# Soltanilara/av-aloha

Measured on AMD Instinct MI355X. Metric: env-steps/sec (whole node) at 4096 parallel envs, SlotInsertion-3Arms, higher is better.
Workload: dtype f32

## Files before the change

av_aloha_amd/build.py:

```python
import os
import subprocess
import sys

HERE = os.path.dirname(os.path.abspath(__file__))
ROOT = os.path.dirname(HERE)
LIB = os.path.join(HERE, "libavsim.so")
SRC = os.path.join(HERE, "csrc")


def _stale(target, sources):
    if not os.path.exists(target):
        return True
    t = os.path.getmtime(target)
    return any(os.path.getmtime(s) > t for s in sources)


def build_hip(force=False, verbose=False):
    srcs = [os.path.join(SRC, f) for f in sorted(os.listdir(SRC)) if not f.endswith(".o") and not f.startswith(".")] + [os.path.join(ROOT, "include", "avsim.h"), os.path.abspath(__file__)]
    if not force and not _stale(LIB, srcs):
        return LIB
    import fcntl
    with open(os.path.join(SRC, ".build.lock"), "w") as lock:
        fcntl.flock(lock, fcntl.LOCK_EX)
        if not force and not _stale(LIB, srcs):
            return LIB
        return _build_hip_locked(verbose)


def _build_hip_locked(verbose):
    hipcc = os.environ.get("HIPCC", "/opt/rocm/bin/hipcc")
    common = [hipcc, "--offload-arch=gfx950", "-std=c++17", "-fPIC", "-fno-gpu-rdc", "-c"]
    units = [
        ("avsim_api", ["-O2", "-fno-hip-fp32-correctly-rounded-divide-sqrt", "-fgpu-flush-denormals-to-zero", "-fno-slp-vectorize", "-fno-vectorize",
                       "-mllvm", "-amdgpu-atomic-optimizer-strategy=None", "-mllvm", "-amdgpu-sched-strategy=max-ilp"] + (["-DAVSIM_RENDER_STATS"] if os.environ.get("AVSIM_RENDER_STATS") else []) + os.environ.get("AVSIM_EXTRA_FLAGS", "").split()),
        ("avsim_phys_f64", ["-O3", "-ffp-contract=off", "-mllvm", "-amdgpu-sched-strategy=max-ilp"] + os.environ.get("AVSIM_EXTRA_FLAGS_F64", "").split()),
    ]
    procs = []
    for name, extra in units:
        cmd = common + extra + ["-o", os.path.join(SRC, name + ".o"), os.path.join(SRC, name + ".hip")]
        if verbose:
            print(" ".join(cmd), file=sys.stderr)
        procs.append((cmd, subprocess.Popen(cmd)))
    for cmd, p in procs:
        if p.wait() != 0:
            raise subprocess.CalledProcessError(p.returncode, cmd)
    tmp = LIB + ".tmp%d" % os.getpid()
    link = [hipcc, "--offload-arch=gfx950", "-shared", "-fPIC", "-fno-gpu-rdc", "-o", tmp] + [os.path.join(SRC, n + ".o") for n, _ in units]
    if verbose:
        print(" ".join(link).replace(tmp, LIB), file=sys.stderr)
    subprocess.check_call(link)
    os.replace(tmp, LIB)
    return LIB


def build_oracle(force=False):
    d = os.path.join(ROOT, "oracle")
    so = os.path.join(d, "liborc.so")
    srcs = [os.path.join(d, f) for f in os.listdir(d) if f.endswith((".c", ".h"))]
    if force or _stale(so, srcs):
        subprocess.check_call(["make", "-C", d, "-B", "liborc.so"], stdout=subprocess.DEVNULL)
    return so


if __name__ == "__main__":
    print(build_hip(force="--force" in sys.argv, verbose=True))
    print(build_oracle(force="--force" in sys.argv))
```

av_aloha_amd/csrc/avsim_api.hip:

```cpp
#include <hip/hip_runtime.h>

#include <cmath>
#include <cstdarg>
#include <cstdio>
#include <cstdlib>
#include <cstring>
#include <memory>
#include <string>
#include <thread>
#include <vector>

#include "../../include/avsim.h"
#include "avsim_compose.hip.h"
#include "avsim_imgprep.hip.h"
#include "avsim_episode.hip.h"
#include "avsim_ik.hip.h"
#include "avsim_jpeg.hip.h"
#include "avsim_model.h"
#include "avsim_phys.hip.h"
#include "avsim_render.hip.h"
#include "avsim_vis.hip.h"

using namespace avs;

// ... 452 lines not shown
    if (!std::strcmp(name, "render_cam_major")) { h->vis.cam_major = value != 0; return AVSIM_OK; }
    if (!std::strcmp(name, "render_chunk")) { if (value < 1) { h->set_error("render_chunk is a number of envs >= 1"); return AVSIM_EINVAL; } h->render.env_chunk = (int)value; return AVSIM_OK; }
    if (!std::strcmp(name, "jpeg_decode_events")) { h->jpegdec_events = value != 0; return AVSIM_OK; }
    if (!std::strcmp(name, "jpeg_decode_budget")) { if (value < 1) { h->set_error("jpeg_decode_budget is a number of bytes >= 1"); return AVSIM_EINVAL; } h->jpegdec.coef_budget = (size_t)value; return AVSIM_OK; }
    if (!std::strcmp(name, "diffik_iters")) { h->ik.diff_iters = (int)value; return AVSIM_OK; }
    if (!std::strcmp(name, "gradik_iters")) { h->ik.grad_iters = (int)value; return AVSIM_OK; }
    try {
        if (h->phys.set_option(name, value)) {
            if (!std::strcmp(name, "num_joints")) h->nj = (int)value;
            return AVSIM_OK;
        }
    } catch (const std::exception& ex) {
        h->set_error("avsim_set_option(%s): %s", name, ex.what());
        return AVSIM_EHIP;
    }
    h->set_error("avsim_set_option: unknown option '%s'", name);
    return AVSIM_EINVAL;
}

int avsim_sync(avsim_t* h) {
    if (!h) return AVSIM_EINVAL;
    AVS_ON_DEVICE(h);
    HIPCHK(h, hipStreamSynchronize(h->stream));
    return AVSIM_OK;
}

int avsim_set_stream(avsim_t* h, void* s) {
    if (!h) return AVSIM_EINVAL;
    AVS_ON_DEVICE(h);
    HIPCHK(h, hipStreamSynchronize(h->stream));
    if (h->own_stream && h->stream) (void)hipStreamDestroy(h->stream);
    h->stream = (hipStream_t)s;
    h->own_stream = false;
    return AVSIM_OK;
}

int avsim_event_record(avsim_t* h, int slot) {
    if (!h || slot < 0 || slot >= 16) return AVSIM_EINVAL;
    AVS_ON_DEVICE(h);
    HIPCHK(h, hipEventRecord(h->ev[slot], h->stream));
    return AVSIM_OK;
}

int avsim_event_elapsed_ms(avsim_t* h, int a, int b, float* ms) {
    if (!h || !ms || a < 0 || a >= 16 || b < 0 || b >= 16) return AVSIM_EINVAL;
    AVS_ON_DEVICE(h);
    HIPCHK(h, hipEventSynchronize(h->ev[b]));
    HIPCHK(h, hipEventElapsedTime(ms, h->ev[a], h->ev[b]));
    return AVSIM_OK;
}

int avsim_kernel_time(avsim_t* h, int reset, double* total_ms, int64_t* launches) {
    if (!h) return AVSIM_EINVAL;
    AVS_ON_DEVICE(h);
    double tot = 0;
    for (size_t i = 0; i + 1 < h->kev_used; i += 2) {
        float ms = 0;
        HIPCHK(h, hipEventSynchronize(h->kev[i + 1]));
        HIPCHK(h, hipEventElapsedTime(&ms, h->kev[i], h->kev[i + 1]));
        tot += ms;
    }
    if (total_ms) *total_ms = tot + h->kev_ms;
    if (launches) *launches = (int64_t)(h->kev_used / 2) + h->kev_n;
    if (reset) { h->kev_used = 0; h->kev_ms = 0; h->kev_n = 0; }
    return AVSIM_OK;
}

int avsim_render_kernel_time(avsim_t* h, int reset, double* total_ms, int64_t* launches) {
    if (!h) return AVSIM_EINVAL;
    AVS_ON_DEVICE(h);
    double tot = 0;
    for (size_t i = 0; i + 1 < h->render.tev_used; i += 2) {
        float ms = 0;
        HIPCHK(h, hipEventSynchronize(h->render.tev[i + 1]));
        HIPCHK(h, hipEventElapsedTime(&ms, h->render.tev[i], h->render.tev[i + 1]));
        tot += ms;
    }
    if (total_ms) *total_ms = tot + h->render.tev_ms;
    if (launches) *launches = (int64_t)(h->render.tev_used / 2) + h->render.tev_n;
    if (reset) { h->render.tev_used = 0; h->render.tev_ms = 0; h->render.tev_n = 0; }
    return AVSIM_OK;
}

int avsim_observe(avsim_t* h, double* agent_pos, int32_t* reward, uint8_t* success) {
    if (!h) return AVSIM_EINVAL;
    AVS_ON_DEVICE(h);
    int rc;
    void *dap = nullptr, *drw = nullptr, *dsu = nullptr;
    size_t N = h->N;
    if (agent_pos && (rc = h->out_begin(4, agent_pos, sizeof(double) * N * h->nj, &dap))) return rc;
    if (reward && (rc = h->out_begin(5, reward, sizeof(int32_t) * N, &drw))) return rc;
    if (success && (rc = h->out_begin(6, success, N, &dsu))) return rc;
    h->phys.force_reward = 1;
    rc = h->phys.launch(h->stream, h->N, 0, nullptr, h->nj, h->d_qpos, h->d_qvel, h->d_ctrl, h->d_warm, h->d_latch, (double*)dap, (int32_t*)drw,
                        (uint8_t*)dsu, h->err);
    h->phys.force_reward = 0;
    if (rc) return rc;
    if ((rc = h->out_end(4, agent_pos, sizeof(double) * N * h->nj))) return rc;
    if ((rc = h->out_end(5, reward, sizeof(int32_t) * N))) return rc;
    if ((rc = h->out_end(6, success, N))) return rc;
    return h->finish();
}

int avsim_fk_jac(avsim_t* h, int arm, int n, const double* q, double* T, double* J) {
    if (!h || arm < 0 || arm > 2 || n <= 0 || !q) { if (h) h->set_error("avsim_fk_jac: bad arguments"); return AVSIM_EINVAL; }
    AVS_ON_DEVICE(h);
    int nj = h->ik.arm[arm].n, rc;
    const void* dq;
    void *dT = nullptr, *dJ = nullptr;
    if ((rc = h->in(0, q, sizeof(double) * n * nj, &dq))) return rc;
    if (T && (rc = h->out_begin(1, T, sizeof(double) * n * 16, &dT))) return rc;
    if (J && (rc = h->out_begin(2, J, sizeof(double) * n * 6 * nj, &dJ))) return rc;
    dim3 grid((n + 63) / 64);
    if (nj == 6) hipLaunchKernelGGL(k_fk_jac<6>, grid, dim3(64), 0, h->stream, h->ik, arm, n, (const double*)dq, (double*)dT, (double*)dJ);
    else hipLaunchKernelGGL(k_fk_jac<7>, grid, dim3(64), 0, h->stream, h->ik, arm, n, (const double*)dq, (double*)dT, (double*)dJ);
    HIPCHK(h, hipGetLastError());
    if ((rc = h->out_end(1, T, sizeof(double) * n * 16))) return rc;
    if ((rc = h->out_end(2, J, sizeof(double) * n * 6 * nj))) return rc;
    return h->finish();
}

int avsim_ik(avsim_t* h, int arm, int controller, int max_iters, int n, const double* q, const double* pos,
             const double* quat, double* qout) {
    if (!h || arm < 0 || arm > 2 || n <= 0 || !q || !pos || !quat || !qout || controller < 0 || controller > 1) {
        if (h) h->set_error("avsim_ik: bad arguments");
        return AVSIM_EINVAL;
    }
    if (controller == 1 && arm == 2) { h->set_error("avsim_ik: GradIK is defined for the 6-DoF manipulators only"); return AVSIM_EINVAL; }
    AVS_ON_DEVICE(h);
    int nj = h->ik.arm[arm].n, rc;
    int iters = max_iters > 0 ? max_iters : (controller == 0 ? h->ik.diff_iters : h->ik.grad_iters);
    const void *dq, *dp, *dqt;
    void* dout;
    if ((rc = h->in(0, q, sizeof(double) * n * nj, &dq))) return rc;
    if ((rc = h->in(1, pos, sizeof(double) * n * 3, &dp))) return rc;
    if ((rc = h->in(2, quat, sizeof(double) * n * 4, &dqt))) return rc;
    if ((rc = h->out_begin(3, qout, sizeof(double) * n * nj, &dout))) return rc;
    dim3 grid(controller == 1 ? (n + 3) / 4 : (n + 63) / 64);
    if (nj == 6)
        hipLaunchKernelGGL(k_ik<6>, grid, dim3(64), 0, h->stream, h->ik, arm, controller, iters, n, (const double*)dq, (const double*)dp,
                           (const double*)dqt, (double*)dout);
    else
        hipLaunchKernelGGL(k_ik<7>, grid, dim3(64), 0, h->stream, h->ik, arm, controller, iters, n, (const double*)dq, (const double*)dp,
                           (const double*)dqt, (double*)dout);
    HIPCHK(h, hipGetLastError());
    if ((rc = h->out_end(3, qout, sizeof(double) * n * nj))) return rc;
    return h->finish();
}

}

template <typename real>
static int reset_impl(avsim_t* h, const uint8_t* mask, const double* obj) {
    int rc;
    const void *dm = nullptr, *dobj;
    if (mask && (rc = h->in(0, mask, h->N, &dm))) return rc;
    if ((rc = h->in(1, obj, sizeof(double) * h->N * h->nobj * 7, &dobj))) return rc;
    hipLaunchKernelGGL(k_reset<real>, dim3((h->N + 63) / 64), dim3(64), 0, h->stream, h->N, h->nq, h->nv, h->nu, h->nobj,
                       (const unsigned char*)dm, (const double*)dobj, h->phys.d_qpos_home, h->phys.d_ctrl_home, h->phys.d_obj_qadr,
                       (real*)h->d_qpos, (real*)h->d_qvel, (real*)h->d_ctrl, (real*)h->d_warm, h->d_latch, h->phys.d_obj_reset);
    HIPCHK(h, hipGetLastError());
    if ((rc = h->phys.launch(h->stream, h->N, 0, nullptr, h->nj, h->d_qpos, h->d_qvel, h->d_ctrl, h->d_warm, h->d_latch, nullptr, nullptr,
                             nullptr, h->err)))
        return rc;
    return h->finish();
}

extern "C" {

int avsim_reset(avsim_t* h, const uint8_t* mask, const double* obj_qpos) {
    if (!h || !obj_qpos) { if (h) h->set_error("avsim_reset: obj_qpos is required"); return AVSIM_EINVAL; }
    AVS_ON_DEVICE(h);
    h->state_ver++;
    return h->f64 ? reset_impl<double>(h, mask, obj_qpos) : reset_impl<float>(h, mask, obj_qpos);
}

static int step_common(avsim_t* h, const float* d_action, int nsub, double* agent_pos, int32_t* reward, uint8_t* success) {
    int rc;
    h->state_ver++;
    void *dap = nullptr, *drw = nullptr, *dsu = nullptr;
    size_t N = h->N;
    if (agent_pos && (rc = h->out_begin(4, agent_pos, sizeof(double) * N * h->nj, &dap))) return rc;
    if (reward && (rc = h->out_begin(5, reward, sizeof(int32_t) * N, &drw))) return rc;
    if (success && (rc = h->out_begin(6, success, N, &dsu))) return rc;
    if (h->ktiming) {
        if (h->kev_used >= 2 * EV_RING) {
            for (size_t i = 0; i + 1 < h->kev_used; i += 2) {
                float ms = 0;
                HIPCHK(h, hipEventSynchronize(h->kev[i + 1]));
                HIPCHK(h, hipEventElapsedTime(&ms, h->kev[i], h->kev[i + 1]));
                h->kev_ms += ms;
            }
            h->kev_n += (int64_t)(h->kev_used / 2);
            h->kev_used = 0;
        }
        while (h->kev.size() < h->kev_used + 2) { hipEvent_t e; HIPCHK(h, hipEventCreate(&e)); h->kev.push_back(e); }
        HIPCHK(h, hipEventRecord(h->kev[h->kev_used], h->stream));
    }
    if ((rc = h->phys.launch(h->stream, h->N, nsub, d_action, h->nj, h->d_qpos, h->d_qvel, h->d_ctrl, h->d_warm, h->d_latch, (double*)dap,
                             (int32_t*)drw, (uint8_t*)dsu, h->err)))
        return rc;
    if (h->ktiming) {
        HIPCHK(h, hipEventRecord(h->kev[h->kev_used + 1], h->stream));
        h->kev_used += 2;
    }
    if ((rc = h->out_end(4, agent_pos, sizeof(double) * N * h->nj))) return rc;
    if ((rc = h->out_end(5, reward, sizeof(int32_t) * N))) return rc;
    if ((rc = h->out_end(6, success, N))) return rc;
    return h->finish();
}

int avsim_step(avsim_t* h, const float* action, int nsub, double* agent_pos, int32_t* reward, uint8_t* success) {
    if (!h || !action || nsub < 0) { if (h) h->set_error("avsim_step: bad arguments"); return AVSIM_EINVAL; }
    AVS_ON_DEVICE(h);
    const void* da;
    int rc;
    if ((rc = h->in(0, action, sizeof(float) * h->N * h->nj, &da))) return rc;
    return step_common(h, (const float*)da, nsub, agent_pos, reward, success);
}

int avsim_step_ctrl(avsim_t* h, int nsub, double* agent_pos, int32_t* reward, uint8_t* success) {
    if (!h || nsub < 0) { if (h) h->set_error("avsim_step_ctrl: bad arguments"); return AVSIM_EINVAL; }
    AVS_ON_DEVICE(h);
    return step_common(h, nullptr, nsub, agent_pos, reward, success);
}

int avsim_step_cartesian(avsim_t* h, const double* action23, int ik_mode, int nsub, double* agent_pos, int32_t* reward,
                         uint8_t* success) {
    if (!h || !action23 || nsub < 0 || (ik_mode != AVSIM_IK_REFERENCE && ik_mode != AVSIM_IK_DLS)) {
        if (h) h->set_error("avsim_step_cartesian: bad arguments");
        return AVSIM_EINVAL;
    }
    if (h->num_arms != 3) { h->set_error("avsim_step_cartesian: the 23-D Cartesian action drives three arms (sim_env.py:277-282)"); return AVSIM_EINVAL; }
    AVS_ON_DEVICE(h);
    const void* da;
    int rc;
    if ((rc = h->in(0, action23, sizeof(double) * h->N * 23, &da))) return rc;
    auto launch = [&](dim3 grid, int arm0) {
        if (h->f64)
            hipLaunchKernelGGL(k_cart_ctrl<double>, grid, dim3(64), 0, h->stream, h->ik, ik_mode, arm0, h->N, h->nq, h->nu, (const double*)da,
                               (const double*)h->d_qpos, (double*)h->d_ctrl);
        else
            hipLaunchKernelGGL(k_cart_ctrl<float>, grid, dim3(64), 0, h->stream, h->ik, ik_mode, arm0, h->N, h->nq, h->nu, (const double*)da,
                               (const float*)h->d_qpos, (float*)h->d_ctrl);
    };
    if (ik_mode == AVSIM_IK_DLS) launch(dim3((h->N + 63) / 64, 3), 0);
    else {
        if (h->f64) hipLaunchKernelGGL(k_gradik_ctrl<double>, dim3((h->N + 3) / 4, 2), dim3(64), 0, h->stream, h->ik, h->N, h->nq, h->nu, (const double*)da, (const double*)h->d_qpos, (double*)h->d_ctrl);
        else hipLaunchKernelGGL(k_gradik_ctrl<float>, dim3((h->N + 3) / 4, 2), dim3(64), 0, h->stream, h->ik, h->N, h->nq, h->nu, (const double*)da, (const float*)h->d_qpos, (float*)h->d_ctrl);
        launch(dim3((h->N + 63) / 64, 1), 2);
    }
    HIPCHK(h, hipGetLastError());
    return step_common(h, nullptr, nsub, agent_pos, reward, success);
}

static int put(avsim_t* h, int slot, const double* src, void* dst, size_t n) {
    if (!src) return 0;
    const void* d;
    int rc;
    if ((rc = h->in(slot, src, sizeof(double) * n, &d))) return rc;
    unsigned g = (unsigned)((n + 255) / 256);
    if (h->f64) hipLaunchKernelGGL((k_convert<double, double>), dim3(g), dim3(256), 0, h->stream, n, (const double*)d, (double*)dst);
    else hipLaunchKernelGGL((k_convert<double, float>), dim3(g), dim3(256), 0, h->stream, n, (const double*)d, (float*)dst);
    return 0;
}
static int get(avsim_t* h, int slot, double* dst, const void* src, size_t n) {
    if (!dst) return 0;
    void* d;
    int rc;
    if ((rc = h->out_begin(slot, dst, sizeof(double) * n, &d))) return rc;
    unsigned g = (unsigned)((n + 255) / 256);
    if (h->f64) hipLaunchKernelGGL((k_convert<double, double>), dim3(g), dim3(256), 0, h->stream, n, (const double*)src, (double*)d);
    else hipLaunchKernelGGL((k_convert<float, double>), dim3(g), dim3(256), 0, h->stream, n, (const float*)src, (double*)d);
    return h->out_end(slot, dst, sizeof(double) * n);
}

int avsim_get_state(avsim_t* h, double* qpos, double* qvel, double* ctrl, double* warm) {
    if (!h) return AVSIM_EINVAL;
    AVS_ON_DEVICE(h);
    size_t N = h->N;
    int rc;
    if ((rc = get(h, 0, qpos, h->d_qpos, N * h->nq))) return rc;
    if ((rc = get(h, 1, qvel, h->d_qvel, N * h->nv))) return rc;
    if ((rc = get(h, 2, ctrl, h->d_ctrl, N * h->nu))) return rc;
    if ((rc = get(h, 3, warm, h->d_warm, N * h->nv))) return rc;
    HIPCHK(h, hipGetLastError());
    return h->finish();
}

int avsim_set_state(avsim_t* h, const double* qpos, const double* qvel, const double* ctrl, const double* warm) {
    if (!h) return AVSIM_EINVAL;
    AVS_ON_DEVICE(h);
    h->state_ver++;
    size_t N = h->N;
    int rc;
    if ((rc = put(h, 0, qpos, h->d_qpos, N * h->nq))) return rc;
    if ((rc = put(h, 1, qvel, h->d_qvel, N * h->nv))) return rc;
    if ((rc = put(h, 2, ctrl, h->d_ctrl, N * h->nu))) return rc;
    if ((rc = put(h, 3, warm, h->d_warm, N * h->nv))) return rc;
    HIPCHK(h, hipGetLastError());
    if ((rc = h->phys.launch(h->stream, h->N, 0, nullptr, h->nj, h->d_qpos, h->d_qvel, h->d_ctrl, h->d_warm, h->d_latch, nullptr, nullptr,
                             nullptr, h->err)))
        return rc;
    return h->finish();
}

int avsim_get_latch(avsim_t* h, int32_t* latch) {
    if (!h || !latch) return AVSIM_EINVAL;
    AVS_ON_DEVICE(h);
    HIPCHK(h, hipMemcpyAsync(latch, h->d_latch, sizeof(int32_t) * (size_t)h->N, h->io_device ? hipMemcpyDeviceToDevice : hipMemcpyDeviceToHost, h->stream));
    return h->finish();
}

int avsim_set_latch(avsim_t* h, const int32_t* latch) {
    if (!h || !latch) return AVSIM_EINVAL;
    AVS_ON_DEVICE(h);
    HIPCHK(h, hipMemcpyAsync(h->d_latch, latch, sizeof(int32_t) * (size_t)h->N, h->io_device ? hipMemcpyDeviceToDevice : hipMemcpyHostToDevice, h->stream));
    return h->finish();
}

int avsim_get_reset_poses(avsim_t* h, double* obj_qpos) {
    if (!h || !obj_qpos) return AVSIM_EINVAL;
    AVS_ON_DEVICE(h);
    HIPCHK(h, hipMemcpyAsync(obj_qpos, h->phys.d_obj_reset, sizeof(double) * (size_t)h->N * h->nobj * 7, h->io_device ? hipMemcpyDeviceToDevice : hipMemcpyDeviceToHost, h->stream));
    return h->finish();
}

int avsim_set_reset_poses(avsim_t* h, const double* obj_qpos) {
    if (!h || !obj_qpos) return AVSIM_EINVAL;
    AVS_ON_DEVICE(h);
    HIPCHK(h, hipMemcpyAsync(h->phys.d_obj_reset, obj_qpos, sizeof(double) * (size_t)h->N * h->nobj * 7, h->io_device ? hipMemcpyDeviceToDevice : hipMemcpyHostToDevice, h->stream));
    return h->finish();
}

int avsim_set_qpos(avsim_t* h, const double* qpos) {
    if (!h || !qpos) return AVSIM_EINVAL;
    return avsim_set_state(h, qpos, nullptr, nullptr, nullptr);
}

int avsim_get_contacts(avsim_t* h, int32_t* ncon, int32_t* pairs, double* dist) {
    if (!h) return AVSIM_EINVAL;
    AVS_ON_DEVICE(h);
    size_t N = h->N, cap = h->phys.maxcon;
    if (h->io_device) {
        if (ncon) HIPCHK(h, hipMemcpyAsync(ncon, h->phys.d_ncon, N * 4, hipMemcpyDeviceToDevice, h->stream));
        if (pairs) HIPCHK(h, hipMemcpyAsync(pairs, h->phys.d_cpairs, N * cap * 8, hipMemcpyDeviceToDevice, h->stream));
        if (dist) HIPCHK(h, hipMemcpyAsync(dist, h->phys.d_cdist, N * cap * 8, hipMemcpyDeviceToDevice, h->stream));
        return AVSIM_OK;
    }
    HIPCHK(h, hipStreamSynchronize(h->stream));
    if (ncon) HIPCHK(h, hipMemcpy(ncon, h->phys.d_ncon, N * 4, hipMemcpyDeviceToHost));
    if (pairs) HIPCHK(h, hipMemcpy(pairs, h->phys.d_cpairs, N * cap * 8, hipMemcpyDeviceToHost));
    if (dist) HIPCHK(h, hipMemcpy(dist, h->phys.d_cdist, N * cap * 8, hipMemcpyDeviceToHost));
    return AVSIM_OK;
}

int avsim_get_phase_cycles(avsim_t* h, int64_t* out) {
    if (!h || !out || !h->phys.d_prof) return AVSIM_EINVAL;
    AVS_ON_DEVICE(h);
    HIPCHK(h, hipStreamSynchronize(h->stream));
    HIPCHK(h, hipMemcpy(out, h->phys.d_prof, (size_t)h->N * avs::PROF_W * 8, h->io_device ? hipMemcpyDeviceToDevice : hipMemcpyDeviceToHost));
    return AVSIM_OK;
}

int avsim_get_diag(avsim_t* h, int32_t* diag) {
    if (!h || !diag) return AVSIM_EINVAL;
    AVS_ON_DEVICE(h);
    size_t N = h->N;
    if (h->io_device) {
        HIPCHK(h, hipMemcpyAsync(diag, h->phys.d_diag, N * 16, hipMemcpyDeviceToDevice, h->stream));
        return AVSIM_OK;
    }
    HIPCHK(h, hipStreamSynchronize(h->stream));
    HIPCHK(h, hipMemcpy(diag, h->phys.d_diag, N * 16, hipMemcpyDeviceToHost));
    return AVSIM_OK;
// ... 497 lines not shown
```

av_aloha_amd/csrc/avsim_newton.hip.h:

```cpp
#pragma once
#include "avsim_math.hip.h"

namespace avs {

typedef float nv4f __attribute__((ext_vector_type(4)));
typedef double nv2d __attribute__((ext_vector_type(2)));
AVS_DEV void load_row16(GLB_PTR(const float) src, float* v) {
    GLB_PTR(const nv4f) p = (GLB_PTR(const nv4f))src;
    nv4f a = p[0], b = p[1], c = p[2], d = p[3];
    asm volatile("" : "+v"(a), "+v"(b), "+v"(c), "+v"(d));
    v[0] = a.x; v[1] = a.y; v[2] = a.z; v[3] = a.w; v[4] = b.x; v[5] = b.y; v[6] = b.z; v[7] = b.w;
    v[8] = c.x; v[9] = c.y; v[10] = c.z; v[11] = c.w; v[12] = d.x; v[13] = d.y; v[14] = d.z; v[15] = d.w;
}
AVS_DEV void load_row16(GLB_PTR(const double) src, double* v) {
    GLB_PTR(const nv2d) p = (GLB_PTR(const nv2d))src;
    nv2d t[8];
#pragma unroll
    for (int q = 0; q < 8; q++) t[q] = p[q];
    asm volatile("" : "+v"(t[0]), "+v"(t[1]), "+v"(t[2]), "+v"(t[3]), "+v"(t[4]), "+v"(t[5]), "+v"(t[6]), "+v"(t[7]));
#pragma unroll
    for (int q = 0; q < 8; q++) { v[2 * q] = t[q].x; v[2 * q + 1] = t[q].y; }
}

template <typename real>
// ... 491 lines not shown
    const int nv = A.nv;
    NComp c;
    c.mydof = lane < nv ? lane : nv; c.nc = nv; c.oa0 = 0; c.on = 0; c.oact = false;
    if (A.ntree > 8 || whole) return c;
    unsigned mine = 0;
    for (int i = lane; i < ne; i += 64) {
        const int ra = A.rowI[i];
        if (((ra >> 19) & 15) != 0) mine |= (1u << ((ra >> 10) & 7)) | (1u << ((ra >> 23) & 7));
    }
    unsigned tmask = 0;
#pragma unroll
    for (int t = 0; t < 8; t++) tmask |= __any((mine >> t) & 1u) ? (1u << t) : 0u;
    const bool isc = lane < nv && ((tmask >> A.dof_tree[lane < nv ? lane : 0]) & 1u);
    const unsigned long long cm = __ballot(isc);
    c.nc = __popcll(cm);
    if (c.nc == nv) return c;
    if (isc) tmp[__popcll(cm & ((1ull << lane) - 1ull))] = lane;
    NSYNC();
    c.mydof = lane < c.nc ? tmp[lane] : nv;
    NSYNC();
    const int t = lane >> 3;
    c.oact = t < A.ntree && !((tmask >> t) & 1u);
    c.oa0 = c.oact ? A.tree_dofadr[t] : 0;
    c.on = c.oact ? A.tree_dofnum[t] : 0;
    return c;
}

template <typename real, bool FWD>
AVS_DEV void ncomp_subst(const NewtonArgs<real>& A, const NComp& c, int lane) {
    const int nv = A.nv, nc = c.nc, i8 = lane & 7;
    const bool omine = c.oact && i8 < c.on;
    const int a0 = c.oa0, obase = (a0 + i8) * (a0 + i8 + 1) / 2 + a0;
    real ocf[TREE_W];
#pragma unroll
    for (int k = 0; k < TREE_W; k++) {
        const bool in = FWD ? (omine && k < i8) : (omine && k < c.on && k > i8);
        const real v = A.H[in ? (FWD ? obase + k : (a0 + k) * (a0 + k + 1) / 2 + a0 + i8) : 0];
        ocf[k] = in ? v : real(0);
    }
    const real odg = A.H[omine ? obase + i8 : 0];
    const real odinv = omine ? real(1) / odg : real(1);
    const real og = A.g[omine ? a0 + i8 : 0];
    real ox = omine ? (FWD ? -og : og) : real(0);
    const int md = c.mydof, rb = md * (md + 1) / 2;
    const bool cm = lane < nc;
    const real cg = A.g[cm ? md : 0];
    real x = cm ? (FWD ? -cg : cg) : real(0);
    const real dinv = cm ? real(1) / A.H[rb + md] : real(0);
    if (nc < nv) {
#pragma unroll
        for (int jj = 0; jj < TREE_W; jj++) {
            const int j = FWD ? jj : TREE_W - 1 - jj;
            const real xj = oct_bcast_n(ox * odinv, j);
            ox = i8 == j ? xj : ox - ocf[j] * xj;
        }
    }
    if (FWD) {
        int cn = __builtin_amdgcn_readlane(md, 0);
        real Lnext = (lane > 0 && cm) ? A.H[rb + cn] : real(0);
        for (int j = 0; j < nc; j++) {
            const real Lc = Lnext;
            if (j + 1 < nc) { cn = __builtin_amdgcn_readlane(md, j + 1); Lnext = (lane > j + 1 && cm) ? A.H[rb + cn] : real(0); }
            const real yj = lane_get(x * dinv, j);
            if (lane == j) x = yj;
            else if (lane > j) x -= Lc * yj;
        }
    } else {
        int cn = __builtin_amdgcn_readlane(md, nc - 1);
        real Lnext = lane < nc - 1 ? A.H[cn * (cn + 1) / 2 + md] : real(0);
        for (int i = nc - 1; i >= 0; i--) {
            const real Lc = Lnext;
            if (i > 0) { cn = __builtin_amdgcn_readlane(md, i - 1); Lnext = lane < i - 1 ? A.H[cn * (cn + 1) / 2 + md] : real(0); }
            const real xi = lane_get(x * dinv, i);
            if (lane == i) x = xi;
            else if (lane < i) x -= Lc * xi;
        }
    }
    NSYNC();
    LDS_PTR(real) out = FWD ? A.g : A.dl;
    if (cm) out[md] = x;
    if (nc < nv && omine) out[a0 + i8] = ox;
}

template <typename real, int NCH, bool COUPLED>
__device__ __attribute__((always_inline)) int newton_solve(KPtr<real> ka, GLB_PTR(const real) rows, LDS_PTR(real) r_, LDS_PTR(int) ii_, LDS_PTR(const int) li_, int nefc, int ncon, int nlead,
                                                      int iters, real tol, real scale, int profiling) {
    const int lane = threadIdx.x & 63;
    NewtonArgs<real> A;
    {
        LDS_PTR(real) r = (LDS_PTR(real))(unsigned long long)(unsigned)__builtin_amdgcn_readfirstlane((int)(unsigned)(unsigned long long)r_);
        LDS_PTR(int) ii = (LDS_PTR(int))(unsigned long long)(unsigned)__builtin_amdgcn_readfirstlane((int)(unsigned)(unsigned long long)ii_);
        LDS_PTR(const int) li = (LDS_PTR(const int))(unsigned long long)(unsigned)__builtin_amdgcn_readfirstlane((int)(unsigned)(unsigned long long)li_);
        tol = lane_get(tol, 0); scale = lane_get(scale, 0);
        const Layout __attribute__((address_space(4)))* L = &ka->lay;
        const MOff __attribute__((address_space(4)))* O = &ka->mo;
        A.rowS = r + L->rowS; A.rowI = ii + L->rowI; A.rmeta = ii + L->rmeta;
        {
            const unsigned long long p_ = (unsigned long long)rows;
            A.rJ = (GLB_PTR(const real))(((unsigned long long)(unsigned)__builtin_amdgcn_readfirstlane((int)(unsigned)(p_ >> 32)) << 32) | (unsigned)__builtin_amdgcn_readfirstlane((int)(unsigned)p_));
        }
        A.M = r + L->M; A.a = r + L->qacc; A.as = r + L->asm_;
        A.H = r + L->nH; A.g = r + L->ng; A.dl = r + L->ndl; A.jv = r + L->njv;
        A.cefc = ii + L->cefc;
        A.prof = profiling ? ii + L->nprof : (LDS_PTR(int))nullptr;
        A.tree_dofadr = li + O->tree_dofadr; A.tree_dofnum = li + O->tree_dofnum; A.tree_madr = li + O->tree_madr; A.dof_tree = li + O->dof_tree;
        A.nv = __builtin_amdgcn_readfirstlane(ka->m.nv); A.ntree = __builtin_amdgcn_readfirstlane(ka->m.ntree);
        A.nefc = __builtin_amdgcn_readfirstlane(nefc); A.ncon = __builtin_amdgcn_readfirstlane(ncon);
        A.nlead = __builtin_amdgcn_readfirstlane(nlead); A.iters = __builtin_amdgcn_readfirstlane(iters);
        A.tol = tol; A.scale = scale; A.ls_tol = ka->m.ls_tolerance; A.ls_iters = __builtin_amdgcn_readfirstlane(ka->m.ls_iterations);
        A.early_exit = __builtin_amdgcn_readfirstlane(ka->m.newton_early_exit);
    }
    const int nv = A.nv, ne = A.nefc;
    {
        const int k = lane < nv ? lane : 0, t = A.dof_tree[k];
        A.k_a0 = A.tree_dofadr[t]; A.k_n = A.tree_dofnum[t]; A.k_mb = A.tree_madr[t] + (k - A.k_a0) * A.k_n;
    }
    int used = 0;
    constexpr bool coupled = COUPLED;
    NComp comp;
    if constexpr (coupled) comp = ncomponent<real>(A, lane, ne, (LDS_PTR(int))A.dl, __builtin_amdgcn_readfirstlane(ka->m.newton_component) == 0);
    long long tp0 = A.prof ? __builtin_readcyclecounter() : 0;
    NCon<real> con[NCH];
#pragma unroll
    for (int ch = 0; ch < NCH; ch++) {
        NCon<real>& c = con[ch];
        const int ci = ch * 64 + lane;
        const int ce = ci < A.ncon ? A.cefc[ci] : -1;
        c.head = ce >= 0 ? (ce & 0xffff) : -1;
        c.dim = ce >= 0 ? (ce >> 16) : 0;
        c.mu = 0; c.Dm = 0;
#pragma unroll
        for (int j = 0; j < 6; j++) { c.S[j] = 0; c.D[j] = 0; }
        if (c.head >= 0) {
#pragma unroll
            for (int j = 0; j < 6; j++)
                if (j < c.dim) { c.D[j] = real(1) / A.rowS[RS_S * (c.head + j) + 1]; if (j > 0) c.S[j] = real(1) / A.rowS[RS_S * (c.head + j) + 7]; }
            if (c.dim > 1) {
                const real R0 = A.rowS[RS_S * c.head + 1], R1 = A.rowS[RS_S * (c.head + 1) + 1];
                c.mu = c.S[1] * sqrt(R1 / R0);
                c.S[0] = c.mu;
                c.Dm = (real(1) / R0) / tmax(real(1e-15), c.mu * c.mu * (1 + c.mu * c.mu));
            }
        }
    }
    const bool jar_ready = true;
    {
        const real c1 = ncost<real, NCH>(A, lane, con, A.as, 8, false);
        const real c0 = ncost<real, NCH>(A, lane, con, (LDS_PTR(const real))A.a, 2);
        if (!(c0 < c1)) {
            for (int k = lane; k < nv; k += 64) A.a[k] = A.as[k];
            for (int i = lane; i < ne; i += 64) A.rowS[RS_S * i + 2] = A.rowS[RS_S * i + 8];
        }
        NSYNC();
    }
    NPROF(0);
    int zone[NCH];
    real cw[NCH][6], cc1[NCH][6], cc2[NCH][6], cs1[NCH], cs2[NCH];
    bool have_L = false;
    unsigned long long sig_lead = 0, sig_z1[NCH];
#pragma unroll
    for (int ch = 0; ch < NCH; ch++) sig_z1[ch] = 0;
    bool forces_current = false, quad_step = false;
    unsigned long long prev_lead = 0, prev_sgn = 0, prev_z1[NCH];
#pragma unroll
    for (int ch = 0; ch < NCH; ch++) prev_z1[ch] = 0;
    real alpha_prev = 0;
    for (int it = 0; it < A.iters; it++) {
        used++;
        if (it > 0) {
            for (int i = lane; i < ne; i += 64) A.rowS[RS_S * i + 2] += alpha_prev * A.jv[i];
            NSYNC();
        } else if (!jar_ready) {
            for (int i = lane; i < ne; i += 64) A.rowS[RS_S * i + 2] = nrow_dot(A, i, (LDS_PTR(const real))A.a) - A.rowS[RS_S * i];
            NSYNC();
        }
        for (int i = lane; i < A.nlead; i += 64) {
            real f, h;
            nrow_scalar<real>(A.rmeta[i] & 3, A.rowS[RS_S * i + 2], A.rowS[RS_S * i + 1], A.rowS[RS_S * i + 5], &f, &h);
            A.rowS[RS_S * i + 6] = f;
            A.jv[i] = h;
        }
#pragma unroll
        for (int ch = 0; ch < NCH; ch++) {
            zone[ch] = 0;
            if (ch * 64 >= A.ncon) break;
            const NCon<real>& c = con[ch];
            if (c.head >= 0) {
                real jar[6], f[6], cc;
// ... 129 lines not shown
        real alpha = 0, lo = 0, hi = -1, dphi0 = 0, dxold = 0, dx = 0;
        for (int ls = 0; ls <= A.ls_iters; ls++) {
            real gsum = 0, hsum = 0;
            for (int i = lane; i < A.nlead; i += 64) {
                real f, h;
                const real jvi = A.jv[i];
                nrow_scalar<real>(A.rmeta[i] & 3, A.rowS[RS_S * i + 2] + alpha * jvi, A.rowS[RS_S * i + 1], A.rowS[RS_S * i + 5], &f, &h);
                gsum -= f * jvi;
                hsum += h * jvi * jvi;
            }
#pragma unroll
            for (int ch = 0; ch < NCH; ch++) {
                if (ch * 64 >= A.ncon) break;
                if (con[ch].head >= 0) {
                    real jar[6], d1, d2;
#pragma unroll
                    for (int j = 0; j < 6; j++) jar[j] = cj0[ch][j] + alpha * cjv[ch][j];
                    ncone_ls(con[ch], jar, cjv[ch], &d1, &d2);
                    gsum += d1;
                    hsum += d2;
                }
            }
            const real dphi = q1 + alpha * q2 + wave_sum(gsum), ddphi = q2 + wave_sum(hsum);
#ifdef AVSIM_DEBUG_NEWTON
            if (lane == 0 && A.iters == 99 && it == 2) printf("         ls %d: alpha %.12e dphi %.6e ddphi %.6e lo %.6e hi %.6e\n", ls, (double)alpha, (double)dphi, (double)ddphi, (double)lo, (double)hi);
#endif
            if (ls == 0) {
                dphi0 = dphi;
                if (!(dphi0 < 0)) break;
                alpha = -dphi0 / ddphi;
                dxold = alpha; dx = alpha;
                continue;
            }
            if (fabs(dphi) < A.ls_tol * fabs(dphi0)) break;
            if (dphi < 0) lo = alpha; else hi = alpha;
            real nx = alpha - dphi / ddphi;
            if (hi < 0) { if (!(nx > lo)) nx = 2 * alpha + real(1e-12); }
            else if (!(nx > lo && nx < hi) || fabs(nx - alpha) > real(0.5) * fabs(dxold)) nx = real(0.5) * (lo + hi);
            dxold = dx;
            dx = nx - alpha;
            if (fabs(nx - alpha) < (sizeof(real) == 8 ? real(1e-14) : real(1e-7)) * (1 + fabs(alpha))) { alpha = nx; break; }
            alpha = nx;
        }
        NPROF(4);
#ifdef AVSIM_DEBUG_NEWTON
        if (lane == 0 && A.iters == 99) printf("      line search: dphi0 %.6e alpha %.6e q1 %.6e q2 %.6e lo %.6e hi %.6e  same-H %d middle %d\n", (double)dphi0, (double)alpha, (double)q1, (double)q2, (double)lo, (double)hi, (int)(same && !middle), (int)middle);
#endif
        if (!(dphi0 < 0)) break;
        real st2 = 0;
        for (int k = lane; k < nv; k += 64) { const real s = alpha * A.dl[k]; A.a[k] += s; st2 += s * s; }
        alpha_prev = alpha;
        st2 = wave_sum(st2);
        NSYNC();
        if (sqrt(st2) * A.scale < real(1e-2) * A.tol) break;
        if (real(-0.5) * alpha * dphi0 * A.scale < A.tol) break;
    }
    if (!forces_current) {
        for (int i = lane; i < ne; i += 64) A.rowS[RS_S * i + 2] = (i < A.nlead ? nrow_dot_lead(A, i, (LDS_PTR(const real))A.a) : nrow_dot(A, i, (LDS_PTR(const real))A.a)) - A.rowS[RS_S * i];
        NSYNC();
        for (int i = lane; i < A.nlead; i += 64) {
            real f, h;
            nrow_scalar<real>(A.rmeta[i] & 3, A.rowS[RS_S * i + 2], A.rowS[RS_S * i + 1], A.rowS[RS_S * i + 5], &f, &h);
            A.rowS[RS_S * i + 6] = f;
        }
    #pragma unroll
        for (int ch = 0; ch < NCH; ch++) {
            if (ch * 64 >= A.ncon) break;
            const NCon<real>& c = con[ch];
            if (c.head >= 0) {
                real jar[6], f[6], w[6], c1[6], c2[6], cc, s1, s2;
    #pragma unroll
                for (int j = 0; j < 6; j++) jar[j] = j < c.dim ? A.rowS[RS_S * (c.head + j) + 2] : real(0);
                ncone(c, jar, f, &cc, w, c1, c2, &s1, &s2);
    #pragma unroll
                for (int j = 0; j < 6; j++) if (j < c.dim) A.rowS[RS_S * (c.head + j) + 6] = f[j];
            }
        }
    }
    NSYNC();
    NPROF(5);
    return used;
}

template <typename real, int NCH>
__device__ AVS_OUTLINE_5 int newton_solve_coupled(KPtr<real> ka, GLB_PTR(const real) rows, LDS_PTR(real) r_, LDS_PTR(int) ii_, LDS_PTR(const int) li_, int nefc, int ncon, int nlead,
                                                              int iters, real tol, real scale, int profiling) {
    return newton_solve<real, NCH, true>(ka, rows, r_, ii_, li_, nefc, ncon, nlead, iters, tol, scale, profiling);
}

}
```

av_aloha_amd/csrc/avsim_phys.hip.h:

```cpp
#pragma once
#include <hip/hip_runtime.h>

#include <string>
#include <vector>

#include "avsim_collide.hip.h"
#include "avsim_math.hip.h"
#include "avsim_model.h"

namespace avs {

enum { J_FREE = 0, J_BALL = 1, J_SLIDE = 2, J_HINGE = 3 };
enum { R_EQ = 0, R_FLOSS = 1, R_LIMIT = 2, R_CONTACT = 3 };
constexpr int TREE_W = 8;
constexpr int ROW_W = 2 * TREE_W;
constexpr int ROW_S = ROW_W;
constexpr int RS_S = 9;
constexpr int CAND_MAX = 256;
constexpr int PROF_W = 26;
constexpr int ANC_MAX = 64;
constexpr int NEAR_MAX = 512;

template <typename real>
struct DevModel {
    int nq, nv, nu, nbody, njnt, ngeom, npair, ntree, neq, nfloss, nlimited, nment, task_id, nj, msize;
    real timestep, gravity[3], impratio, grip_lo, grip_hi;
    int noslip_iters;
    int noslip_trees;
    int qcqp_tridiag;
    int newton_early_exit;
    int newton_component;
    int noslip_per_tree;
    int solver, newton_iters;
    real newton_tol, nscale;
    real ls_tolerance;
    int ls_iterations;
    GLB_PTR(const int) body_parent;
    GLB_PTR(const int) body_jntadr;
    GLB_PTR(const int) body_jntnum;
    GLB_PTR(const int) body_dofadr;
    GLB_PTR(const int) body_dofnum;
    GLB_PTR(const int) body_tree;
    GLB_PTR(const int) body_dofmask;
    GLB_PTR(const int) body_last;
    GLB_PTR(const real) body_pos;
    GLB_PTR(const real) body_quat;
    GLB_PTR(const real) body_mass;
    GLB_PTR(const real) body_ipos;
    GLB_PTR(const real) body_inertia;
    GLB_PTR(const real) body_invweight0;
    GLB_PTR(const real) static_xpos;
    GLB_PTR(const real) static_xmat;
    GLB_PTR(const int) tree_bodyadr;
    GLB_PTR(const int) tree_bodylist;
    GLB_PTR(const int) tree_dofadr;
    GLB_PTR(const int) tree_dofnum;
    GLB_PTR(const int) tree_madr;
    GLB_PTR(const int) jnt_type;
    GLB_PTR(const int) jnt_qposadr;
    GLB_PTR(const int) jnt_dofadr;
    GLB_PTR(const int) jnt_actfrclimited;
    GLB_PTR(const int) limited_jnt;
    GLB_PTR(const real) jnt_pos;
    GLB_PTR(const real) jnt_axis;
    GLB_PTR(const real) jnt_range;
    GLB_PTR(const real) jnt_actfrcrange;
    GLB_PTR(const real) jnt_solref;
    GLB_PTR(const real) jnt_solimp;
    GLB_PTR(const real) jnt_margin;
    GLB_PTR(const int) dof_body;
    GLB_PTR(const int) dof_parent;
    GLB_PTR(const int) dof_tree;
    GLB_PTR(const int) dof_jnt;
    GLB_PTR(const int) floss_dof;
    GLB_PTR(const int) ment_i;
    GLB_PTR(const int) ment_j;
    GLB_PTR(const real) dof_armature;
    GLB_PTR(const real) dof_damping;
    GLB_PTR(const real) dof_frictionloss;
    GLB_PTR(const real) dof_invweight0;
    GLB_PTR(const real) dof_solref;
    GLB_PTR(const real) dof_solimp;
    GLB_PTR(const int) act_dof;
    GLB_PTR(const int) act_qposadr;
    GLB_PTR(const int) act_ctrllimited;
    GLB_PTR(const real) act_kp;
    GLB_PTR(const real) act_kv;
    GLB_PTR(const real) act_gear;
    GLB_PTR(const real) act_ctrlrange;
    GLB_PTR(const int) eq_dof1;
    GLB_PTR(const int) eq_dof2;
    GLB_PTR(const int) eq_qpos1;
    GLB_PTR(const int) eq_qpos2;
    GLB_PTR(const real) eq_polycoef;
    GLB_PTR(const real) eq_solref;
    GLB_PTR(const real) eq_solimp;
    GLB_PTR(const real) qpos0;
    GLB_PTR(const real) qpos_home;
    int nobj;
    GLB_PTR(const int) obj_qadr;
    const double* obj_reset;
    GLB_PTR(const int) geom_type;
    GLB_PTR(const int) geom_body;
    GLB_PTR(const int) geom_hull;
    GLB_PTR(const int) geom_class;
    GLB_PTR(const int) geom_static;
    GLB_PTR(const real) geom_pos;
    GLB_PTR(const real) geom_mat;
    GLB_PTR(const real) geom_size;
    GLB_PTR(const real) geom_cpos;
    GLB_PTR(const real) geom_rbound;
    GLB_PTR(const real) geom_xpos0;
    GLB_PTR(const real) geom_xmat0;
    GLB_PTR(const real) geom_cen0;
    GLB_PTR(const real) geom_aabb0;
    GLB_PTR(const real) geom_lbox;
    GLB_PTR(const real) hull_vert;
    int hull_ovf;
    GLB_PTR(const int) pair_geom;
    GLB_PTR(const int) pair_condim;
    GLB_PTR(const real) pair_friction;
    GLB_PTR(const real) pair_solref;
    GLB_PTR(const real) pair_solimp;
    GLB_PTR(const real) pair_margin;
    GLB_PTR(const real) pair_gap;
    real* rJ_glob;
    real* rB_glob;
    real* gA_glob;
    int* near_glob;
    int* cand_glob;
    real* gref_glob;
    real* bxo_glob;
    GLB_PTR(const int) obs_qposadr;
    GLB_PTR(const real) obs_offset;
    GLB_PTR(const real) obs_scale;
};

struct MOff {
    int nreal, nint;
    int body_parent;
    int body_jntadr;
    int body_jntnum;
    int body_dofadr;
    int body_dofnum;
    int body_tree;
    int body_dofmask;
    int body_last;
    int tree_bodyadr;
    int tree_bodylist;
    int tree_dofadr;
    int tree_dofnum;
    int tree_madr;
    int jnt_type;
    int jnt_qposadr;
    int jnt_dofadr;
    int jnt_actfrclimited;
    int limited_jnt;
    int dof_body;
    int dof_parent;
    int dof_tree;
    int dof_jnt;
    int floss_dof;
    int ment_i;
    int ment_j;
    int act_dof;
    int act_qposadr;
    int act_ctrllimited;
    int geom_type;
    int geom_body;
    int geom_static;
    int body_pos;
    int body_quat;
    int body_mass;
    int body_ipos;
    int body_inertia;
    int body_invweight0;
    int jnt_pos;
    int jnt_axis;
    int jnt_range;
    int jnt_actfrcrange;
    int jnt_margin;
    int dof_armature;
    int dof_damping;
    int dof_frictionloss;
    int dof_invweight0;
    int act_kp;
    int act_kv;
    int act_gear;
    int act_ctrlrange;
    int geom_cpos;
    int geom_rbound;
};

struct Layout {
    int qpos, qvel, ctrl, warm, xpos, xmat, xipos, cdof, gcen, M, L, Minv, bias, fsm, asm_, qacc, fcon, nH, ng, ndl, njv, U, nreal;
    int cinert, cvel, cacc, cfrc, binert;
    int cdist, cpos, cnrm, rowS, scr;
    int cand, cpair, cefc, rmeta, rowI, gI, misc, nprof, nint;
    int maxgrp;
    int maxcon, maxefc;
    int expcon;
    int gefc, ggrp;
    int bytes_per_env;
};

template <typename real>
struct KArgs {
    DevModel<real> m;
    Layout lay;
    MOff mo;
};
template <typename real>
using KPtr = const KArgs<real> __attribute__((address_space(4)))*;
#define PHASE_LAUNDER()                                                                                \
    do {                                                                                               \
        const unsigned long long p_ = (unsigned long long)ka;                                          \
        unsigned lo_ = __builtin_amdgcn_readfirstlane((unsigned)p_), hi_ = __builtin_amdgcn_readfirstlane((unsigned)(p_ >> 32)); \
        asm volatile("" : "+s"(lo_), "+s"(hi_));                                                       \
        ka = (decltype(ka))(((unsigned long long)hi_ << 32) | lo_);                                    \
    } while (0)
#if defined(__HIP_DEVICE_COMPILE__)
#define AVS_ASSUME_LDS(p) __builtin_assume(__builtin_amdgcn_is_shared((const void*)(p)))
#else
#define AVS_ASSUME_LDS(p) ((void)(p))
#endif
#define LDS_BASES()                                                                       \
    real* const r = this->r; AVS_ASSUME_LDS(r);     \
    int* const ii = this->ii; AVS_ASSUME_LDS(ii);   \
    (void)r; (void)ii
#define PHASE_BEGIN() PHASE_LAUNDER(); LDS_BASES()



#ifndef AVS_SYNC_SCOPE
#define AVS_SYNC_SCOPE "workgroup"
#endif
#define GSYNC()                                              \
    do {                                                     \
        __builtin_amdgcn_fence(__ATOMIC_ACQ_REL, AVS_SYNC_SCOPE); \
        __builtin_amdgcn_wave_barrier();                     \
    } while (0)

AVS_DEV float row16_sum(float x) {
    asm volatile("" : "+v"(x));
    x += __builtin_bit_cast(float, __builtin_amdgcn_mov_dpp(__builtin_bit_cast(int, x), 0x128, 0xf, 0xf, true));
    x += __builtin_bit_cast(float, __builtin_amdgcn_mov_dpp(__builtin_bit_cast(int, x), 0x124, 0xf, 0xf, true));
    x += __builtin_bit_cast(float, __builtin_amdgcn_mov_dpp(__builtin_bit_cast(int, x), 0x122, 0xf, 0xf, true));
    x += __builtin_bit_cast(float, __builtin_amdgcn_mov_dpp(__builtin_bit_cast(int, x), 0x121, 0xf, 0xf, true));
    return x;
}
AVS_DEV double row16_sum(double x) {
    x += __shfl_xor(x, 8, 16);
    x += __shfl_xor(x, 4, 16);
    x += __shfl_xor(x, 2, 16);
    x += __shfl_xor(x, 1, 16);
    return x;
}

AVS_DEV float wave_sum(float x) {
    x = row16_sum(x);
    int xi = __builtin_bit_cast(int, x);
    x += __builtin_bit_cast(float, __builtin_amdgcn_update_dpp(0, xi, 0x142, 0xa, 0xf, false));
    xi = __builtin_bit_cast(int, x);
    x += __builtin_bit_cast(float, __builtin_amdgcn_update_dpp(0, xi, 0x143, 0xc, 0xf, false));
    return __builtin_bit_cast(float, __builtin_amdgcn_readlane(__builtin_bit_cast(int, x), 63));
}
AVS_DEV double wave_sum(double x) {
    for (int o = 32; o > 0; o >>= 1) x += __shfl_xor(x, o, 64);
    return x;
}

#define LDS_PTR(T) __attribute__((address_space(3))) T*

template <typename real>
struct RowS {
    real aref, R, inv, invn, lo, hi, f, muinv;
};

AVS_DEV float oct_sum(float x) {
    asm volatile("" : "+v"(x));
    x += __builtin_bit_cast(float, __builtin_amdgcn_mov_dpp(__builtin_bit_cast(int, x), 0xB1, 0xf, 0xf, true));
    x += __builtin_bit_cast(float, __builtin_amdgcn_mov_dpp(__builtin_bit_cast(int, x), 0x4E, 0xf, 0xf, true));
    x += __builtin_bit_cast(float, __builtin_amdgcn_mov_dpp(__builtin_bit_cast(int, x), 0x141, 0xf, 0xf, true));
    return x;
}
AVS_DEV double oct_sum(double x) {
    x += __shfl_xor(x, 1, 8);
    x += __shfl_xor(x, 2, 8);
    x += __shfl_xor(x, 4, 8);
    return x;
}
template <int J>
AVS_DEV int oct_bcast_i(int x) {
    constexpr int q = J & 3, ctrl = q | (q << 2) | (q << 4) | (q << 6);
    const int a = __builtin_amdgcn_mov_dpp(x, ctrl, 0xf, 0xf, true);
    const int b = __builtin_amdgcn_mov_dpp(a, 0x141, 0xf, 0xf, true);
// ... 1083 lines not shown
                    if (fi == 1) f = v0;
                    if (fi == 2) f = v1;
                }
            }
            const real dl = row ? f - cur.f0 : real(0);
#pragma unroll
            for (int r = 1; r < GRP_MAX; r++) x += (r < dim ? cur.B[r] : real(0)) * oct_bcast_n(dl, r);
            if (row && cur.side == 0) rowS[RS_S * (cur.h + fi) + 8] = f;
        };
        rem = chain;
        fetch(0, ca);
        for (int step = 0; step < nstep; step += 2) {
            fetch(step + 1, cb);
            one_step(ca);
            if (step + 1 < nstep) {
                fetch(step + 2, ca);
                one_step(cb);
            }
        }
        if (__any(slid)) { if (prof && lane == 0) prof[2] += 1; return 0; }
        __builtin_amdgcn_fence(__ATOMIC_ACQ_REL, "wavefront");
        __builtin_amdgcn_wave_barrier();
        if (lane_get(wave_sum(imp), 0) < noslip_tol_scaled) break;
    }
    return 1;
    };
    if (!(__any(tB >= 0) ? sweeps(BoolTag<true>{}) : sweeps(BoolTag<false>{}))) return 0;
    if (prof && lane == 0) prof[3] += 1;
    if (fm) q[fdof] = x;
    if (frow >= 0) FS[8] = ff;
    __builtin_amdgcn_fence(__ATOMIC_ACQ_REL, "wavefront");
    __builtin_amdgcn_wave_barrier();
    for (int i = lane; i < nefc; i += 64) rowS[RS_S * i + 6] = rowS[RS_S * i + 8];
    __builtin_amdgcn_fence(__ATOMIC_ACQ_REL, "wavefront");
    __builtin_amdgcn_wave_barrier();
    return 1;
}


}
#include "avsim_newton.hip.h"
namespace avs {

typedef float avs_v4f __attribute__((ext_vector_type(4)));
typedef double avs_v2d __attribute__((ext_vector_type(2)));
AVS_DEV void store_row16(GLB_PTR(float) dst, const float* v) {
#pragma unroll
    for (int q = 0; q < 4; q++) { avs_v4f t = {v[4 * q], v[4 * q + 1], v[4 * q + 2], v[4 * q + 3]}; ((GLB_PTR(avs_v4f))dst)[q] = t; }
}
AVS_DEV void store_row16(GLB_PTR(double) dst, const double* v) {
#pragma unroll
    for (int q = 0; q < 8; q++) { avs_v2d t = {v[2 * q], v[2 * q + 1]}; ((GLB_PTR(avs_v2d))dst)[q] = t; }
}

AVS_DEV void lds_load8(const float* p, float* v) {
    LDS_PTR(const avs_v4f) q = (LDS_PTR(const avs_v4f))p;
    const avs_v4f a = q[0], b = q[1];
    v[0] = a.x; v[1] = a.y; v[2] = a.z; v[3] = a.w; v[4] = b.x; v[5] = b.y; v[6] = b.z; v[7] = b.w;
}
AVS_DEV void lds_load8(const double* p, double* v) {
    LDS_PTR(const avs_v2d) q = (LDS_PTR(const avs_v2d))p;
#pragma unroll
    for (int k = 0; k < 4; k++) { const avs_v2d a = q[k]; v[2 * k] = a.x; v[2 * k + 1] = a.y; }
}

template <int G>
AVS_DEV unsigned long long group_mask(int grp) {
    if (G == 64) return ~0ull;
    return ((1ull << G) - 1ull) << (grp * G);
}
template <int G>
AVS_DEV int group_rank(bool flag, int grp, int lane, int* total) {
    unsigned long long b = __ballot(flag) & group_mask<G>(grp);
    unsigned long long lower = (G == 64) ? ((1ull << lane) - 1ull) : (((1ull << lane) - 1ull) << (grp * G));
    *total = __popcll(b);
    return __popcll(b & lower);
}

template <typename real>
struct SInert {
    real m, h[3], I[6];
};

template <typename real>
AVS_DEV void body_inertia(KPtr<real> ka, const real* xmat, const real* xipos, int b, SInert<real>& s) {
    const real* R = xmat + 9 * b;
    GLB_PTR(const real) Ib = ka->m.body_inertia + 6 * b;
    real I3[9] = {Ib[0], Ib[3], Ib[4], Ib[3], Ib[1], Ib[5], Ib[4], Ib[5], Ib[2]}, T[9], Ic[9];
#pragma unroll
    for (int i = 0; i < 3; i++)
#pragma unroll
        for (int j = 0; j < 3; j++) T[3 * i + j] = R[3 * i] * I3[j] + R[3 * i + 1] * I3[3 + j] + R[3 * i + 2] * I3[6 + j];
#pragma unroll
    for (int i = 0; i < 3; i++)
#pragma unroll
        for (int j = 0; j < 3; j++) Ic[3 * i + j] = T[3 * i] * R[3 * j] + T[3 * i + 1] * R[3 * j + 1] + T[3 * i + 2] * R[3 * j + 2];
    real ms = ka->m.body_mass[b];
    real c[3] = {xipos[3 * b], xipos[3 * b + 1], xipos[3 * b + 2]};
    real cc = dot3(c, c);
    s.m = ms;
    s.h[0] = ms * c[0]; s.h[1] = ms * c[1]; s.h[2] = ms * c[2];
    s.I[0] = Ic[0] + ms * (cc - c[0] * c[0]); s.I[1] = Ic[4] + ms * (cc - c[1] * c[1]); s.I[2] = Ic[8] + ms * (cc - c[2] * c[2]);
    s.I[3] = Ic[1] - ms * c[0] * c[1]; s.I[4] = Ic[2] - ms * c[0] * c[2]; s.I[5] = Ic[5] - ms * c[1] * c[2];
}

template <typename real>
AVS_DEV void inert_mul(const real* s , const real* mv, real* f) {
    const real *w = mv, *v = mv + 3, *h = s + 1, *I = s + 4;
    real hv[3], hw[3];
    cross3(h, v, hv);
    cross3(h, w, hw);
    f[0] = I[0] * w[0] + I[3] * w[1] + I[4] * w[2] + hv[0];
    f[1] = I[3] * w[0] + I[1] * w[1] + I[5] * w[2] + hv[1];
    f[2] = I[4] * w[0] + I[5] * w[1] + I[2] * w[2] + hv[2];
    f[3] = s[0] * v[0] - hw[0]; f[4] = s[0] * v[1] - hw[1]; f[5] = s[0] * v[2] - hw[2];
}

template <typename real>
AVS_DEV void cross_motion(const real* v, const real* s, real* o) {
    real a[3], b[3], c[3];
    cross3(v, s, a);
    cross3(v, s + 3, b);
    cross3(v + 3, s, c);
    o[0] = a[0]; o[1] = a[1]; o[2] = a[2];
    o[3] = b[0] + c[0]; o[4] = b[1] + c[1]; o[5] = b[2] + c[2];
}
template <typename real>
AVS_DEV void cross_force(const real* v, const real* f, real* o) {
    real a[3], b[3], c[3];
    cross3(v, f, a);
    cross3(v + 3, f + 3, b);
    cross3(v, f + 3, c);
    o[0] = a[0] + b[0]; o[1] = a[1] + b[1]; o[2] = a[2] + b[2];
    o[3] = c[0]; o[4] = c[1]; o[5] = c[2];
}

template <typename real>
AVS_DEV void chol_block(const real* A, real* L, int n) {
    for (int j = 0; j < n; j++) {
        real dd = A[j * n + j];
        for (int k = 0; k < j; k++) dd -= L[j * n + k] * L[j * n + k];
        dd = sqrt(tmax(dd, real(1e-30)));
        L[j * n + j] = dd;
        real inv = real(1) / dd;
        for (int i = j + 1; i < n; i++) {
            real s = A[i * n + j];
            for (int k = 0; k < j; k++) s -= L[i * n + k] * L[j * n + k];
            L[i * n + j] = s * inv;
        }
    }
}
template <typename real>
AVS_DEV void chol_solve_block(const real* L, real* x, int n) {
    for (int i = 0; i < n; i++) {
        real s = x[i];
        for (int k = 0; k < i; k++) s -= L[i * n + k] * x[k];
        x[i] = s / L[i * n + i];
    }
    for (int i = n - 1; i >= 0; i--) {
        real s = x[i];
        for (int k = i + 1; k < n; k++) s -= L[k * n + i] * x[k];
        x[i] = s / L[i * n + i];
    }
}

template <typename real>
AVS_DEV real imp_pow(real x, real p) { return p == real(2) ? x * x : pow(x, p); }
template <typename real>
AVS_DEV real impedance(const real* si, real pos, real margin) {
    real dmin = tclamp(si[0], real(0.0001), real(0.9999)), dmax = tclamp(si[1], real(0.0001), real(0.9999));
    real width = tmax(si[2], real(1e-15)), mid = tclamp(si[3], real(0.0001), real(0.9999)), power = tmax(si[4], real(1));
    if (dmin == dmax) return real(0.5) * (dmin + dmax);
    real x = fabs(pos - margin) / width;
    if (x >= 1) return dmax;
    if (x <= 0) return dmin;
    real y;
    if (power == 1) y = x;
    else if (x <= mid) y = imp_pow(x / mid, power) * mid;
    else y = 1 - imp_pow((1 - x) / (1 - mid), power) * (1 - mid);
    return dmin + y * (dmax - dmin);
}

AVS_DEV int has_pair(int c1, int c2, int a, int b) { return ((c1 & a) && (c2 & b)) || ((c2 & a) && (c1 & b)); }
AVS_DEV int reward_pair_flags(int c1, int c2, int t) {
    enum { CL = 1, CR = 2, CT = 4, CA = 8, CB = 16, CC = 32, CD = 64 };
    int f = 0;
    if (has_pair(c1, c2, CT, CA)) f |= 4;
    if (has_pair(c1, c2, CT, CB)) f |= 8;
    if (has_pair(c1, c2, CA, CB)) f |= 16;
    if (has_pair(c1, c2, CC, CD)) f |= 32;
    if (has_pair(c1, c2, CA, CD)) f |= 64;
    if (has_pair(c1, c2, CA, CC)) f |= 128;
    if (has_pair(c1, c2, CA, CR)) f |= 2;
    if (t == 0 || t == 3) { if (has_pair(c1, c2, CB, CL)) f |= 1; }
    else { if (has_pair(c1, c2, CA, CL)) f |= 1; }
    return f;
}
AVS_DEV int reward_from_flags(int f, int t, int* latch) {
    bool tl = f & 1, tr = f & 2, a_table = f & 4, b_table = f & 8, ab = f & 16, cd = f & 32, ad = f & 64, ac = f & 128;
    int rw = 0;
    switch (t) {
        case 0:
            if (tl && tr) rw = 1;
            if (tl && tr && !a_table && !b_table) rw = 2;
            if (ab && !a_table && !b_table) rw = 3;
            if (ac) rw = 4;
            break;
        case 1:
            if (tl && tr) rw = 1;
            if (tl && tr && !a_table) rw = 2;
            if (ab && !a_table) rw = 3;
            if (cd) rw = 4;
            break;
        case 2:
            if (cd) *latch = 1;
            if (tr) rw = 1;
            if (tr && !a_table) rw = 2;
            if (ab && !a_table) rw = 3;
            if (*latch) rw = 4;
            if (tl && !tr && !a_table && !ad && *latch) rw = 5;
            break;
        case 3:
            if (tl && tr) rw = 1;
            if (tl && tr && !a_table && !b_table) rw = 2;
            if (cd) rw = 3;
            break;
        default:
            if (tl && tr) rw = 1;
            if (tl && tr && !a_table) rw = 2;
            if (ab && !a_table) rw = 3;
            if (cd) rw = 4;
    }
    return rw;
}
#ifndef AVSIM_TU_F64
__global__ void k_reward_pairs(GLB_PTR(const int) geom_class, int ngeom, int task_id, const int* __restrict__ pairs, int n, int cap, int* __restrict__ latch, int* __restrict__ reward) {
    const int i = blockIdx.x * blockDim.x + threadIdx.x;
    if (i >= n) return;
    int f = 0;
    for (int c = 0; c < cap; c++) {
        const int g1 = pairs[((size_t)i * cap + c) * 2], g2 = pairs[((size_t)i * cap + c) * 2 + 1];
        if (g1 < 0 || g2 < 0 || g1 >= ngeom || g2 >= ngeom) continue;
        f |= reward_pair_flags(geom_class[g1], geom_class[g2], task_id);
    }
    int l = latch ? latch[i] : 0;
    reward[i] = reward_from_flags(f, task_id, &l);
    if (latch) latch[i] = l;
}
#endif


template <typename real, int G>
struct Env {
    KPtr<real> ka;
    int env = 0;
    int diverged = 0;
    int nit_sum = 0, nit_max = 0;
    bool profiling = false;
    real* r;
    int* ii;
    int lane, grp;
    const real* lr;
    const int* li;
    long long t_broad = 0, t_narrow = 0;
    __device__ Env(KPtr<real> ka_, real* r_, int* i_, int lane_, int grp_, const real* lr_, const int* li_)
        : ka(ka_), r(r_), ii(i_), lane(lane_), grp(grp_), lr(lr_), li(li_) {}
    AVS_DEV const int* LI() const { const int* p = li; AVS_ASSUME_LDS(p); return p; }
    AVS_DEV const real* LR() const { const real* p = lr; AVS_ASSUME_LDS(p); return p; }
    AVS_DEV GLB_PTR(real) rows_() const { return (GLB_PTR(real))ka->m.rJ_glob + (size_t)env * ka->lay.gefc * ROW_S; }
    AVS_DEV GLB_PTR(real) rowsB_() const { return (GLB_PTR(real))ka->m.rB_glob + (size_t)env * ka->lay.gefc * ROW_S; }
    AVS_DEV GLB_PTR(real) coup_() const { return (GLB_PTR(real))ka->m.gA_glob + (size_t)env * ka->lay.ggrp * GA_W; }
    AVS_DEV GLB_PTR(int) near_() const { return (GLB_PTR(int))ka->m.near_glob + (size_t)env * NEAR_MAX; }
    AVS_DEV GLB_PTR(int) cand_() const { return (GLB_PTR(int))ka->m.cand_glob + (size_t)env * CAND_MAX; }
    AVS_DEV GLB_PTR(real) bxo_() const { return (GLB_PTR(real))ka->m.bxo_glob + (size_t)env * 64 * BOX_OVF_W; }
    AVS_DEV GLB_PTR(real) gref_() const { return (GLB_PTR(real))ka->m.gref_glob + (size_t)env * ka->m.ngeom * 3; }
    AVS_DEV const int* body_parent_() const { return LI() + ka->mo.body_parent; }
    AVS_DEV const int* body_jntadr_() const { return LI() + ka->mo.body_jntadr; }
    AVS_DEV const int* body_jntnum_() const { return LI() + ka->mo.body_jntnum; }
    AVS_DEV const int* body_dofadr_() const { return LI() + ka->mo.body_dofadr; }
    AVS_DEV const int* body_dofnum_() const { return LI() + ka->mo.body_dofnum; }
    AVS_DEV const int* body_tree_() const { return LI() + ka->mo.body_tree; }
    AVS_DEV const int* body_dofmask_() const { return LI() + ka->mo.body_dofmask; }
    AVS_DEV const int* body_last_() const { return LI() + ka->mo.body_last; }
    AVS_DEV const int* tree_bodyadr_() const { return LI() + ka->mo.tree_bodyadr; }
    AVS_DEV const int* tree_bodylist_() const { return LI() + ka->mo.tree_bodylist; }
    AVS_DEV const int* tree_dofadr_() const { return LI() + ka->mo.tree_dofadr; }
    AVS_DEV const int* tree_dofnum_() const { return LI() + ka->mo.tree_dofnum; }
    AVS_DEV const int* tree_madr_() const { return LI() + ka->mo.tree_madr; }
    AVS_DEV const int* jnt_type_() const { return LI() + ka->mo.jnt_type; }
    AVS_DEV const int* jnt_qposadr_() const { return LI() + ka->mo.jnt_qposadr; }
    AVS_DEV const int* jnt_dofadr_() const { return LI() + ka->mo.jnt_dofadr; }
    AVS_DEV const int* jnt_actfrclimited_() const { return LI() + ka->mo.jnt_actfrclimited; }
    AVS_DEV const int* limited_jnt_() const { return LI() + ka->mo.limited_jnt; }
    AVS_DEV const int* dof_body_() const { return LI() + ka->mo.dof_body; }
    AVS_DEV const int* dof_parent_() const { return LI() + ka->mo.dof_parent; }
    AVS_DEV const int* dof_tree_() const { return LI() + ka->mo.dof_tree; }
    AVS_DEV const int* dof_jnt_() const { return LI() + ka->mo.dof_jnt; }
    AVS_DEV const int* floss_dof_() const { return LI() + ka->mo.floss_dof; }
    AVS_DEV const int* ment_i_() const { return LI() + ka->mo.ment_i; }
    AVS_DEV const int* ment_j_() const { return LI() + ka->mo.ment_j; }
    AVS_DEV const int* act_dof_() const { return LI() + ka->mo.act_dof; }
    AVS_DEV const int* act_qposadr_() const { return LI() + ka->mo.act_qposadr; }
    AVS_DEV const int* act_ctrllimited_() const { return LI() + ka->mo.act_ctrllimited; }
    AVS_DEV const int* geom_type_() const { return LI() + ka->mo.geom_type; }
    AVS_DEV const int* geom_body_() const { return LI() + ka->mo.geom_body; }
    AVS_DEV const int* geom_static_() const { return LI() + ka->mo.geom_static; }
    AVS_DEV const real* body_pos_() const { return LR() + ka->mo.body_pos; }
    AVS_DEV const real* body_quat_() const { return LR() + ka->mo.body_quat; }
    AVS_DEV const real* body_mass_() const { return LR() + ka->mo.body_mass; }
    AVS_DEV const real* body_ipos_() const { return LR() + ka->mo.body_ipos; }
    AVS_DEV const real* body_inertia_() const { return LR() + ka->mo.body_inertia; }
    AVS_DEV const real* body_invweight0_() const { return LR() + ka->mo.body_invweight0; }
    AVS_DEV const real* jnt_pos_() const { return LR() + ka->mo.jnt_pos; }
    AVS_DEV const real* jnt_axis_() const { return LR() + ka->mo.jnt_axis; }
    AVS_DEV const real* jnt_range_() const { return LR() + ka->mo.jnt_range; }
    AVS_DEV const real* jnt_actfrcrange_() const { return LR() + ka->mo.jnt_actfrcrange; }
    AVS_DEV const real* jnt_margin_() const { return LR() + ka->mo.jnt_margin; }
    AVS_DEV const real* dof_armature_() const { return LR() + ka->mo.dof_armature; }
    AVS_DEV const real* dof_damping_() const { return LR() + ka->mo.dof_damping; }
    AVS_DEV const real* dof_frictionloss_() const { return LR() + ka->mo.dof_frictionloss; }
    AVS_DEV const real* dof_invweight0_() const { return LR() + ka->mo.dof_invweight0; }
    AVS_DEV const real* act_kp_() const { return LR() + ka->mo.act_kp; }
    AVS_DEV const real* act_kv_() const { return LR() + ka->mo.act_kv; }
    AVS_DEV const real* act_gear_() const { return LR() + ka->mo.act_gear; }
    AVS_DEV const real* act_ctrlrange_() const { return LR() + ka->mo.act_ctrlrange; }
    AVS_DEV const real* geom_cpos_() const { return LR() + ka->mo.geom_cpos; }
    AVS_DEV const real* geom_rbound_() const { return LR() + ka->mo.geom_rbound; }


    __device__ void tree_chol(const real* A, real* Ldst, const real* diag_add, real diag_scale) {
        const int t = lane >> 3, i = lane & 7, gb = lane & ~7;
        const bool act = t < ka->m.ntree;
        const int n = act ? tree_dofnum_()[t] : 0, base = act ? tree_madr_()[t] : 0, a0 = act ? tree_dofadr_()[t] : 0;
        real row[TREE_W];
#pragma unroll
        for (int k = 0; k < TREE_W; k++) row[k] = (i < n && k <= i) ? A[base + i * n + k] : (k == i ? real(1) : real(0));
        if (diag_add && i < n) {
#pragma unroll
            for (int k = 0; k < TREE_W; k++) if (k == i) row[k] += diag_scale * diag_add[a0 + i];
        }
#pragma unroll
        for (int j = 0; j < TREE_W; j++) {
            const real d = sqrt(tmax(oct_bcast_n(row[j], j), real(1e-30)));
            const real lij = i == j ? d : row[j] / d;
            row[j] = lij;
            const real mul = i > j ? lij : real(0);
#pragma unroll
            for (int k = j + 1; k < TREE_W; k++) row[k] -= mul * oct_bcast_n(lij, k);
// ... 297 lines not shown
                real sv[10];
                for (int q = 0; q < 10; q++) sv[q] = (r + ka->lay.binert)[10 * b + q];
                real Ia[6], Iv[6], vIv[6];
                inert_mul(sv, a, Ia);
                inert_mul(sv, v, Iv);
                cross_force(v, Iv, vIv);
                for (int q = 0; q < 6; q++) f[q] = Ia[q] + vIv[q];
            }
            for (int q = 0; q < 6; q++) cfrc[6 * b + q] = f[q];
        }
        GSYNC();
        for (int i = lane; i < ka->m.nv; i += G) {
            const int b = dof_body_()[i];
            real f[6] = {0, 0, 0, 0, 0, 0};
            for (int d = b; d <= body_last_()[b]; d++)
                for (int q = 0; q < 6; q++) f[q] += cfrc[6 * d + q];
            real sacc = 0;
            for (int q = 0; q < 6; q++) sacc += cdof[6 * i + q] * f[q];
            bias[i] = sacc;
        }
        GSYNC();
    }

    __device__ void smooth() {
        PHASE_BEGIN();
        real *qpos = r + ka->lay.qpos, *qvel = r + ka->lay.qvel, *ctrl = r + ka->lay.ctrl, *bias = r + ka->lay.bias, *fsm = r + ka->lay.fsm, *as = r + ka->lay.asm_;
        real* act = r + ka->lay.fcon;
        for (int i = lane; i < ka->m.nv; i += G) act[i] = 0;
        GSYNC();
        for (int u = lane; u < ka->m.nu; u += G) {
            real c = ctrl[u];
            if (act_ctrllimited_()[u]) c = tclamp(c, act_ctrlrange_()[2 * u], act_ctrlrange_()[2 * u + 1]);
            int dof = act_dof_()[u];
            real f = act_kp_()[u] * c - act_kp_()[u] * qpos[act_qposadr_()[u]] - act_kv_()[u] * qvel[dof];
            act[dof] += act_gear_()[u] * f;
        }
        GSYNC();
        for (int i = lane; i < ka->m.nv; i += G) {
            int j = dof_jnt_()[i];
            real a = act[i];
            if (jnt_actfrclimited_()[j] && jnt_type_()[j] != J_FREE) a = tclamp(a, jnt_actfrcrange_()[2 * j], jnt_actfrcrange_()[2 * j + 1]);
            real f = -dof_damping_()[i] * qvel[i] - bias[i] + a;
            fsm[i] = f;
            as[i] = f;
        }
        GSYNC();
        {
            const int t = lane >> 3, i = lane & 7;
            const bool mine = t < ka->m.ntree && i < tree_dofnum_()[t];
            const int k = mine ? tree_dofadr_()[t] + i : 0;
            const real x = tree_solve(r + ka->lay.L, mine ? as[k] : real(0));
            GSYNC();
            if (mine) as[k] = x;
        }
        GSYNC();
    }

    __device__ void load_shape(int g, Shape<real>& s) {
        LDS_BASES();
        real *xpos = r + ka->lay.xpos, *xmat = r + ka->lay.xmat, *gcen = r + ka->lay.gcen;
        s.type = geom_type_()[g];
        for (int k = 0; k < 3; k++) s.size[k] = ka->m.geom_size[3 * g + k];
        s.hull = ka->m.hull_vert;
        s.hbase = ka->m.geom_hull[2 * g];
        s.hR = ka->m.geom_hull[2 * g + 1];
        s.hovf = ka->m.hull_ovf;
        s.nh = 0;
        for (int k = 0; k < 3; k++) { s.lc[k] = ka->m.geom_lbox[6 * g + k]; s.lh[k] = ka->m.geom_lbox[6 * g + 3 + k]; }
        if (geom_static_()[g]) {
            for (int k = 0; k < 3; k++) { s.pos[k] = ka->m.geom_xpos0[3 * g + k]; s.center[k] = ka->m.geom_cen0[3 * g + k]; }
            for (int k = 0; k < 9; k++) s.mat[k] = ka->m.geom_xmat0[9 * g + k];
        } else {
            int b = geom_body_()[g];
            real gp[3] = {ka->m.geom_pos[3 * g], ka->m.geom_pos[3 * g + 1], ka->m.geom_pos[3 * g + 2]}, t3[3];
            mulmat(xmat + 9 * b, gp, t3);
            for (int k = 0; k < 3; k++) { s.pos[k] = xpos[3 * b + k] + t3[k]; s.center[k] = gcen[3 * g + k]; }
            const real* Rb = xmat + 9 * b;
            GLB_PTR(const real) Rg = ka->m.geom_mat + 9 * g;
            for (int i = 0; i < 3; i++)
                for (int j = 0; j < 3; j++) s.mat[3 * i + j] = Rb[3 * i] * Rg[j] + Rb[3 * i + 1] * Rg[3 + j] + Rb[3 * i + 2] * Rg[6 + j];
        }
    }

    __device__ AVS_OUTLINE_0 static void multi_perturb(KPtr<real> ka_, real* r_, int* i_, int lane_, int grp_, const real* lr_, const int* li_, int env_,
                                                                   int pga, int pgb, int src, int pert) {
        Env e(ka_, r_, i_, lane_, grp_, lr_, li_);
        e.env = env_;
        LDS_PTR(real) os = (LDS_PTR(real))(e.r + e.ka->lay.scr + SLOT_W * src);
        const real p0[3] = {os[SLOT_P], os[SLOT_P + 1], os[SLOT_P + 2]}, n0[3] = {os[SLOT_N], os[SLOT_N + 1], os[SLOT_N + 2]};
        Shape<real> a, b;
        e.load_shape(pga, a);
        e.load_shape(pgb, b);
        real dk = real(1e30), pk[3] = {0, 0, 0};
        if (!mpr_perturbed(a, b, p0, n0, pert, &dk, pk)) dk = real(1e30);
        os[1 + pert] = dk;
        for (int c = 0; c < 3; c++) os[SLOT_P + 3 * (1 + pert) + c] = pk[c];
    }

    __device__ AVS_OUTLINE void collide() {
        Env e(*this);
        e.collide_i();
        diverged = e.diverged; nit_sum = e.nit_sum; nit_max = e.nit_max; t_broad = e.t_broad; t_narrow = e.t_narrow;
    }
    __device__ __attribute__((always_inline)) void collide_i() {
        PHASE_BEGIN();
        real* gcen = r + ka->lay.gcen;
        int* misc = ii + ka->lay.misc;
        GLB_PTR(int) cand = cand_();
        int ncand = 0;
        long long tb0 = __builtin_readcyclecounter();
        const real skin = real(0.03);
        GLB_PTR(real) gref = gref_();
        GLB_PTR(int) nearl = near_();
        auto pair_hit = [&](int p, real pad) -> bool {
            int g1 = ka->m.pair_geom[2 * p], g2 = ka->m.pair_geom[2 * p + 1];
            bool s1 = geom_static_()[g1], s2 = geom_static_()[g2];
            real mg = ka->m.pair_margin[p] + pad;
            if (s1 || s2) {
                int gs = s1 ? g1 : g2, gd = s1 ? g2 : g1;
                real rd = geom_rbound_()[gd] + mg, d2 = 0;
                for (int k = 0; k < 3; k++) {
                    real c = gcen[3 * gd + k], lo = ka->m.geom_aabb0[6 * gs + k], hi = ka->m.geom_aabb0[6 * gs + 3 + k];
                    real e = c < lo ? lo - c : (c > hi ? c - hi : real(0));
                    d2 += e * e;
                }
                return !(d2 > rd * rd);
            }
            real d[3], rr = geom_rbound_()[g1] + geom_rbound_()[g2] + mg;
            sub3(gcen + 3 * g2, gcen + 3 * g1, d);
            return !(dot3(d, d) > rr * rr);
        };
        bool moved = false;
        if (misc[7]) {
            for (int g = lane; g < ka->m.ngeom; g += G)
                if (!geom_static_()[g]) {
                    const real d[3] = {gcen[3 * g] - gref[3 * g], gcen[3 * g + 1] - gref[3 * g + 1], gcen[3 * g + 2] - gref[3 * g + 2]};
                    moved |= dot3(d, d) > real(0.25) * skin * skin;
                }
        }
        bool rebuild = !misc[7] || __any(moved);
        int nnear = misc[6];
        if (rebuild) {
            nnear = 0;
            for (int base = 0; base < ka->m.npair; base += G) {
                int p = base + lane;
                bool hit = p < ka->m.npair && pair_hit(p, skin);
                int tot, rk = group_rank<G>(hit, grp, lane, &tot);
                if (hit && nnear + rk < NEAR_MAX) nearl[nnear + rk] = p;
                nnear += tot;
            }
            for (int i = lane; i < 3 * ka->m.ngeom; i += G) gref[i] = gcen[i];
            if (lane == 0) { misc[6] = nnear < NEAR_MAX ? nnear : NEAR_MAX; misc[7] = nnear <= NEAR_MAX; if (nnear > NEAR_MAX) misc[2] |= 8; }
            GSYNC();
        }
        if (nnear <= NEAR_MAX) {
            for (int base = 0; base < nnear; base += G) {
                int i = base + lane, p = i < nnear ? nearl[i] : 0;
                bool hit = i < nnear && pair_hit(p, real(0));
                int tot, rk = group_rank<G>(hit, grp, lane, &tot);
                if (hit && ncand + rk < CAND_MAX) cand[ncand + rk] = p;
                if (ncand + tot > CAND_MAX && lane == 0) misc[2] |= 4;
                ncand = ncand + tot < CAND_MAX ? ncand + tot : CAND_MAX;
            }
        } else {
            for (int base = 0; base < ka->m.npair; base += G) {
                int p = base + lane;
                bool hit = p < ka->m.npair && pair_hit(p, real(0));
// ... 626 lines not shown

    __device__ void check_divergence() {
        LDS_BASES();
        real *qpos = r + ka->lay.qpos, *qvel = r + ka->lay.qvel, *warm = r + ka->lay.warm;
        bool bad = false;
        for (int i = lane; i < ka->m.nq; i += G) bad |= !(fabs(qpos[i]) < real(1e6));
        for (int i = lane; i < ka->m.nv; i += G) bad |= !(fabs(qvel[i]) < real(1e6));
        if (!__any(bad)) return;
        diverged = 1;
        for (int i = lane; i < ka->m.nq; i += G) qpos[i] = ka->m.qpos_home[i];
        GSYNC();
        for (int i = lane; i < ka->m.nobj * 7; i += G) qpos[ka->m.obj_qadr[i / 7] + i % 7] = (real)ka->m.obj_reset[((size_t)env * ka->m.nobj) * 7 + i];
        for (int i = lane; i < ka->m.nv; i += G) { qvel[i] = 0; warm[i] = 0; }
        if (lane == 0) (ii + ka->lay.misc)[7] = 0;
        GSYNC();
    }

    __device__ __attribute__((always_inline)) void jt_force(real* out, int nefc) {
        LDS_BASES();
        AVS_ASSUME_LDS(out);
        (void)nefc;
        int* misc = ii + ka->lay.misc;
        for (int k = lane; k < ka->m.nv; k += G) out[k] = 0;
        GSYNC();
        rows_jt_force<real>((LDS_PTR(const real))(r + ka->lay.rowS), (LDS_PTR(const int))(ii + ka->lay.rowI), (LDS_PTR(const int))(ii + ka->lay.cefc),
                            (GLB_PTR(const real))rows_(), (LDS_PTR(real))out, misc[4], misc[0], lane, real(1));
        GSYNC();
    }

    __device__ void euler() {
        PHASE_BEGIN();
        real *qpos = r + ka->lay.qpos, *qvel = r + ka->lay.qvel, *warm = r + ka->lay.warm, *qacc = r + ka->lay.qacc, *fsm = r + ka->lay.fsm, *fcon = r + ka->lay.fcon;
        real *M = r + ka->lay.M, *L = r + ka->lay.L, *tmp = r + ka->lay.bias;
        real h = ka->m.timestep;
        for (int i = lane; i < ka->m.nv; i += G) { tmp[i] = fsm[i] + fcon[i]; warm[i] = qacc[i]; }
        GSYNC();
        tree_chol(M, L, dof_damping_(), h);
        GSYNC();
        {
            const int t = lane >> 3, i = lane & 7;
            const bool mine = t < ka->m.ntree && i < tree_dofnum_()[t];
            const int k = mine ? tree_dofadr_()[t] + i : 0;
            const real x = tree_solve(L, mine ? tmp[k] : real(0));
            if (mine) qvel[k] += h * x;
        }
        GSYNC();
        for (int j = lane; j < ka->m.njnt; j += G) {
            int qa = jnt_qposadr_()[j], da = jnt_dofadr_()[j];
            if (jnt_type_()[j] == J_FREE) {
                for (int k = 0; k < 3; k++) qpos[qa + k] += h * qvel[da + k];
                real q[4] = {qpos[qa + 3], qpos[qa + 4], qpos[qa + 5], qpos[qa + 6]}, w[3] = {qvel[da + 3], qvel[da + 4], qvel[da + 5]};
                real wn = sqrt(dot3(w, w)), ang = h * wn;
                if (ang > 0) {
                    real s = sin(ang / 2) / wn, qr[4] = {cos(ang / 2), s * w[0], s * w[1], s * w[2]};
                    quatmul(q, qr, q);
                }
                quatnorm(q);
                for (int k = 0; k < 4; k++) qpos[qa + 3 + k] = q[k];
            } else {
                qpos[qa] += h * qvel[da];
            }
        }
        GSYNC();
    }

    __device__ int reward(int* latch) {
        PHASE_BEGIN();
        int *misc = ii + ka->lay.misc, *cpair = ii + ka->lay.cpair;
        int ncon = misc[0];
        int f = 0;
        const int t = ka->m.task_id;
        for (int c = lane; c < ncon; c += G) {
            int p = cpair[c];
            f |= reward_pair_flags(ka->m.geom_class[ka->m.pair_geom[2 * p]], ka->m.geom_class[ka->m.pair_geom[2 * p + 1]], t);
        }
        for (int o = 1; o < G; o <<= 1) f |= __shfl_xor(f, o, G);
        return reward_from_flags(f, t, latch);
    }
};

#ifndef AVSIM_PHYS_MAXW
#define AVSIM_PHYS_MAXW 8
#endif
template <typename real, int G, int MAXW, bool RETRY>
#ifndef AVSIM_PHYS_ATTR
#ifdef AVSIM_TU_F64
#define AVSIM_PHYS_ATTR
#else
#define AVSIM_PHYS_ATTR __attribute__((amdgpu_waves_per_eu(2)))
#endif
#endif
__global__ void __launch_bounds__(64 * MAXW) AVSIM_PHYS_ATTR k_phys(KPtr<real> ka_small, const real* __restrict__ img_real, const int* __restrict__ img_int, int N, int nsub, int pgs_iters, const float* __restrict__ action,
                                             int want_reward, real* __restrict__ g_qpos, real* __restrict__ g_qvel, real* __restrict__ g_ctrl,
                                             real* __restrict__ g_warm, int* __restrict__ g_latch, double* __restrict__ o_agent,
                                             int* __restrict__ o_reward, unsigned char* __restrict__ o_success, int* __restrict__ o_ncon,
                                             int* __restrict__ o_cpairs, double* __restrict__ o_cdist, int* __restrict__ o_diag, int max_reward, int export_contacts, long long* __restrict__ o_prof, float* __restrict__ o_xpose,
                                             const int* __restrict__ env_order, int* __restrict__ o_cost, int* __restrict__ work_head, int* __restrict__ work_next,
                                             int* __restrict__ retry, int retry_mode, KPtr<real> ka_big) {
    extern __shared__ __attribute__((aligned(16))) unsigned char smem[];
    int nwork = N;
    const bool pass2 = RETRY && ((retry_mode & 7) == 2 || (retry_mode & 7) == 4);
    const bool pass1 = RETRY && ((retry_mode & 7) == 1 || (retry_mode & 7) == 3);
    if (pass2) {
        nwork = retry[(retry_mode & 7) == 4];
        if (blockIdx.x == 0 && threadIdx.x == 0) { *work_next = 0; retry[(retry_mode & 7) == 2] = 0; }
        if (nwork <= 0) return;
    }
    int* const bigflag = retry + 2 + N;
    const int cap1_con = pass2 ? (retry_mode >> 8) & 0x3ff : ka_small->lay.maxcon, cap1_efc = pass2 ? (retry_mode >> 18) & 0x3ff : ka_small->lay.maxefc;
    int* const pair_want = reinterpret_cast<int*>(smem + (size_t)(blockDim.x >> 6) * ka_small->lay.bytes_per_env + (size_t)ka_small->mo.nreal * sizeof(real) + (size_t)ka_small->mo.nint * 4);
    int* const pair_grant = pair_want + MAXW / 2;
    if (RETRY && threadIdx.x < MAXW / 2) { pair_want[threadIdx.x] = 0; pair_grant[threadIdx.x] = 0; }
    static_assert(G == 64, "one env per wavefront");
#ifdef AVSIM_NO_PROF
    o_prof = nullptr;
#endif
    const int wpb = blockDim.x >> 6;
    const int wave = threadIdx.x >> 6, lane = threadIdx.x & 63, grp = 0;
    real* lr = reinterpret_cast<real*>(smem + (size_t)wpb * ka_small->lay.bytes_per_env);
    int* li = reinterpret_cast<int*>(lr + ka_small->mo.nreal);
    for (int i = threadIdx.x; i < ka_small->mo.nreal; i += blockDim.x) lr[i] = img_real[i];
    for (int i = threadIdx.x; i < ka_small->mo.nint; i += blockDim.x) li[i] = img_int[i];
    if (blockIdx.x == 0 && threadIdx.x == 0) *work_next = 0;
    __syncthreads();
    const int pr = wave >> 1;
    const bool paired = pass1 && (retry_mode & 8) && (wave | 1) < wpb;
    auto lds_get = [&](int* p) { int v = 0; if (lane == 0) v = __hip_atomic_load(p, __ATOMIC_ACQUIRE, __HIP_MEMORY_SCOPE_WORKGROUP); return __builtin_amdgcn_readfirstlane(v); };
    auto lds_put = [&](int* p, int v) { if (lane == 0) __hip_atomic_store(p, v, __ATOMIC_RELEASE, __HIP_MEMORY_SCOPE_WORKGROUP); };
    auto to_list = [&](int e) { if (lane == 0) retry[2 + atomicAdd(retry + ((retry_mode & 7) == 3), 1)] = e; };
    constexpr int PAIR_LEFT = -1;
    int claim_gen = 0, my_claim = 0;
    auto park = [&]() {
        for (;;) {
            const int w = lds_get(&pair_want[pr]);
            if (w == 0 || (w & 0xff) == wave + 1) break;
            lds_put(&pair_grant[pr], w);
            __builtin_amdgcn_s_sleep(32);
        }
    };
    auto claim = [&]() {
        int got = 0;
        const int c = (++claim_gen << 8) | (wave + 1);
        if (lane == 0) { int expect = 0; got = __hip_atomic_compare_exchange_strong(&pair_want[pr], &expect, c, __ATOMIC_ACQ_REL, __ATOMIC_ACQUIRE, __HIP_MEMORY_SCOPE_WORKGROUP) ? 1 : 0; }
        my_claim = c;
        return __builtin_amdgcn_readfirstlane(got) != 0;
    };
    int redo_env = -1;
  for (;;) {
    int env_ = 0;
    bool big = false;
    if (RETRY && redo_env >= 0) { env_ = redo_env; redo_env = -1; big = true; }
    else {
        if (RETRY && paired) park();
        int slot = 0;
        if (lane == 0) slot = atomicAdd(work_head, 1);
        slot = __builtin_amdgcn_readfirstlane(slot);
        if (slot >= nwork) break;
        env_ = env_order ? env_order[slot] : slot;
        if (RETRY && pass1 && (retry_mode & 8)) big = __builtin_amdgcn_readfirstlane(bigflag[env_]) != 0;
    }
    const int env = env_;
    if (RETRY && big) {
        bool mine = false;
        if (paired) mine = claim();
        if (!mine && paired) {
            for (int tries = 0; tries < 64 && !mine; tries++) {
                park();
                mine = claim();
            }
        }
        if (!mine) { to_list(env); continue; }
        int polls = 0;
        for (;; polls++) {
            const int g = lds_get(&pair_grant[pr]);
            if (g == my_claim || g == PAIR_LEFT || polls >= (1 << 15)) break;
            __builtin_amdgcn_s_sleep(32);
        }
        if (polls >= (1 << 15)) { lds_put(&pair_want[pr], 0); to_list(env); continue; }
    }
    KPtr<real> ka = (RETRY && big) ? ka_big : ka_small;
    const long long t_launch = __builtin_readcyclecounter();
    real* r = reinterpret_cast<real*>(smem + (size_t)((RETRY && big) ? (wave & ~1) : wave) * ka_small->lay.bytes_per_env);
    int* ii = reinterpret_cast<int*>(r + ka->lay.nreal);
    bool beyond = false;
    Env<real, G> E(ka, r, ii, lane, grp, lr, li);
    E.env = env;

    for (int i = lane; i < ka->m.nq; i += G) r[ka->lay.qpos + i] = g_qpos[(size_t)env * ka->m.nq + i];
    for (int i = lane; i < ka->m.nv; i += G) { r[ka->lay.qvel + i] = g_qvel[(size_t)env * ka->m.nv + i]; r[ka->lay.warm + i] = g_warm[(size_t)env * ka->m.nv + i]; }
    for (int i = lane; i < ka->m.nu; i += G) r[ka->lay.ctrl + i] = g_ctrl[(size_t)env * ka->m.nu + i];
    if (lane == 0) for (int k = 0; k < 8; k++) { ii[ka->lay.misc + k] = 0; ii[ka->lay.nprof + k] = 0; ii[ka->lay.nprof + 8 + k] = 0; }
    if (lane == 0) ii[ka->lay.misc + 8] = 0;
    E.profiling = o_prof != nullptr;
    GSYNC();
    if (action) {
        const float* a = action + (size_t)env * ka->m.nj;
        for (int i = lane; i < ka->m.nj; i += G) {
            real v = (real)a[i];
            if (i == 6 || i == 13) v = v * (ka->m.grip_hi - ka->m.grip_lo) + ka->m.grip_lo;
            r[ka->lay.ctrl + i] = v;
        }
        GSYNC();
    }
    long long tp[9] = {0, 0, 0, 0, 0, 0, 0, 0, 0};
#define PROF(k, stmt) do { if (o_prof) { long long t0_ = __builtin_readcyclecounter(); stmt; tp[k] += __builtin_readcyclecounter() - t0_; } else { stmt; } } while (0)
    for (int s = 0; s < nsub; s++) {
#ifndef AVS_NO_SPLIT_PRE
        PROF(0, E.pre_phases());
#else
        {
            Env<real, G> e(E);
            PROF(0, e.kinematics());
            PROF(1, e.crb());
            PROF(2, e.rne_bias());
            PROF(3, e.smooth());
        }
#endif
        PROF(4, E.collide());
        PROF(5, E.make_constraints());
        if (RETRY) beyond = beyond || ii[ka->lay.misc + 0] > cap1_con || ii[ka->lay.misc + 1] > cap1_efc;
        PROF(6, E.solve(pgs_iters, ka->m.solver, ka->m.newton_iters, ka->m.newton_tol, ka->m.nscale));
#ifndef AVS_NO_SPLIT_PRE
        PROF(7, E.post_phases());
#else
        {
            Env<real, G> e(E);
            PROF(7, e.euler());
            e.check_divergence();
            E.diverged = e.diverged;
        }
#endif
    }
    if (o_prof && lane == 0) {
        for (int k = 0; k < 8; k++) o_prof[(size_t)env * PROF_W + k] = tp[k];
        o_prof[(size_t)env * PROF_W + 8] = E.t_broad; o_prof[(size_t)env * PROF_W + 9] = E.t_narrow;
        for (int k = 0; k < 16; k++) o_prof[(size_t)env * PROF_W + 10 + k] = ii[ka->lay.nprof + k];
    }
    int nefc_last = ii[ka->lay.misc + 1];
    E.kinematics();
    if (o_xpose) {
        for (int b = lane; b < ka->m.nbody; b += G) {
            float* o = o_xpose + ((size_t)env * ka->m.nbody + b) * 12;
            for (int k = 0; k < 3; k++) o[k] = (float)r[ka->lay.xpos + 3 * b + k];
            for (int k = 0; k < 9; k++) o[3 + k] = (float)r[ka->lay.xmat + 9 * b + k];
        }
    }
    E.collide();
    if (RETRY && pass1 && !big && (ii[ka->lay.misc + 2] & 3)) {
        if (paired) redo_env = env; else to_list(env);
        GSYNC();
        continue;
    }
    if (RETRY) {
        beyond = beyond || ii[ka->lay.misc + 0] > cap1_con;
        if (lane == 0 && (big || pass2 || (retry_mode & 8))) bigflag[env] = beyond ? 1 : 0;
    }

    if (nsub > 0) {
        for (int i = lane; i < ka->m.nq; i += G) g_qpos[(size_t)env * ka->m.nq + i] = r[ka->lay.qpos + i];
        for (int i = lane; i < ka->m.nv; i += G) { g_qvel[(size_t)env * ka->m.nv + i] = r[ka->lay.qvel + i]; g_warm[(size_t)env * ka->m.nv + i] = r[ka->lay.warm + i]; }
    }
    if (action) for (int i = lane; i < ka->m.nu; i += G) g_ctrl[(size_t)env * ka->m.nu + i] = r[ka->lay.ctrl + i];
    if (o_agent)
        for (int i = lane; i < ka->m.nj; i += G) o_agent[(size_t)env * ka->m.nj + i] = ((double)r[ka->lay.qpos + ka->m.obs_qposadr[i]] - (double)ka->m.obs_offset[i]) * (double)ka->m.obs_scale[i];
    int ncon = ii[ka->lay.misc + 0];
    if (want_reward) {
        int latch = g_latch[env];
        int rw = E.reward(&latch);
        if (lane == 0) {
            g_latch[env] = latch;
            if (o_reward) o_reward[env] = rw;
            if (o_success) o_success[env] = (rw == max_reward);
        }
    }
    if (export_contacts)
    {
    const int expcon = RETRY ? ka->lay.expcon : ka->lay.maxcon;
    for (int c = lane; c < expcon; c += G) {
        int p = c < ncon ? ii[ka->lay.cpair + c] : -1;
        o_cpairs[((size_t)env * expcon + c) * 2] = p >= 0 ? ka->m.pair_geom[2 * p] : -1;
        o_cpairs[((size_t)env * expcon + c) * 2 + 1] = p >= 0 ? ka->m.pair_geom[2 * p + 1] : -1;
        o_cdist[(size_t)env * expcon + c] = c < ncon ? (double)r[ka->lay.cdist + c] : 0.0;
    }
    }
    if (lane == 0 && o_cost && nsub > 0) o_cost[env] = (int)((__builtin_readcyclecounter() - t_launch) >> 6);
    if (lane == 0 && !o_xpose) {
        o_ncon[env] = ncon;
        bool bad = E.diverged != 0;
        for (int i = 0; i < ka->m.nq; i++) bad |= !(fabs(r[ka->lay.qpos + i]) < real(1e6));
        o_diag[4 * env] = ncon; o_diag[4 * env + 1] = nefc_last; o_diag[4 * env + 2] = ii[ka->lay.misc + 2]; o_diag[4 * env + 3] = (bad ? 1 : 0) | ((ii[ka->lay.misc + 3] & 0xff) << 8) | ((E.nit_sum & 0xfff) << 16) | ((E.nit_max < 15 ? E.nit_max : 15) << 28);
    }
    GSYNC();
    if (RETRY && big && pass1) {
        lds_put(&pair_want[pr], 0);
    }
  }
    if (RETRY && paired) lds_put(&pair_grant[pr], PAIR_LEFT);
}

static __global__ void __launch_bounds__(1024) k_env_order(const int* __restrict__ cost, int* __restrict__ order, int N) {
    __shared__ int lo, hi, cnt[256], off[256];
    if (threadIdx.x == 0) { lo = 0x7fffffff; hi = 0; }
    if (threadIdx.x < 256) cnt[threadIdx.x] = 0;
    __syncthreads();
    int mn = 0x7fffffff, mx = 0;
    for (int i = threadIdx.x; i < N; i += 1024) { const int c = cost[i]; mn = c < mn ? c : mn; mx = c > mx ? c : mx; }
    atomicMin(&lo, mn);
    atomicMax(&hi, mx);
    __syncthreads();
    const int base = lo;
    const float scale = 255.0f / (float)(hi - lo + 1);
    auto bucket = [&](int c) { const int b = 255 - (int)((float)(c - base) * scale); return b < 0 ? 0 : (b > 255 ? 255 : b); };
    for (int i = threadIdx.x; i < N; i += 1024) atomicAdd(&cnt[bucket(cost[i])], 1);
    __syncthreads();
    if (threadIdx.x == 0) { int a = 0; for (int b = 0; b < 256; b++) { off[b] = a; a += cnt[b]; } }
    __syncthreads();
    for (int i = threadIdx.x; i < N; i += 1024) order[atomicAdd(&off[bucket(cost[i])], 1)] = i;
}

struct PhysHost;
int phys_launch_f64(PhysHost& ph, hipStream_t st, int nsub, const float* action, void* qpos, void* qvel, void* ctrl, void* warm, int* latch,
                    double* agent, int32_t* reward, uint8_t* success, std::string& err);

struct PhysHost {
    int maxcon = 48, maxefc = 144, pgs_iters = 20, group = 64, export_contacts = 1, force_reward = 0, wpb_override = 0;
    int maxcon1 = 48, maxefc1 = 144;
    bool f64 = false;
    int N = 0, max_reward = 0;
    std::vector<void*> allocs;
    DevModel<float> mf;
    DevModel<double> md;
    Layout lay, lay2;
    bool two_pass() const { return maxcon1 < maxcon || maxefc1 < maxefc; }
    int pair_waves = 1;
    int* d_retry = nullptr;
    unsigned long long retry_parity = 0;
    void* d_kargs2 = nullptr;
    double *d_qpos_home = nullptr, *d_ctrl_home = nullptr, *d_obj_reset = nullptr;
    int* d_obj_qadr = nullptr;
    int *d_ncon = nullptr, *d_cpairs = nullptr, *d_diag = nullptr;
    int *d_cost = nullptr, *d_order = nullptr;
    int order_envs = 1;
    bool have_cost = false;
    long long* d_prof = nullptr;
    float* d_xpose = nullptr;
    double* d_cdist = nullptr;

    std::vector<int> img_int;
    std::vector<double> img_real;
    MOff moff;
    void* d_img_real = nullptr;
    int* d_img_int = nullptr;
    void* d_kargs = nullptr;
    bool kargs_dirty = true;
    unsigned attr_done = 0;
    int num_cu = 256;
    int persist_over = 1;
    int* d_head = nullptr;
    unsigned long long launch_count = 0;
    template <typename T>
    struct DevPtr {
        T* p;
        operator T*() const { return p; }
        operator GLB_PTR(T)() const { return (GLB_PTR(T))p; }
        operator GLB_PTR(const T)() const { return (GLB_PTR(const T))p; }
    };
    template <typename T>
    DevPtr<T> up(const std::vector<T>& v) {
        void* p = nullptr;
        size_t n = (v.size() ? v.size() : 1) * sizeof(T);
        if (hipMalloc(&p, n) != hipSuccess) throw std::runtime_error("hipMalloc failed while uploading the model");
        if (v.size() && hipMemcpy(p, v.data(), v.size() * sizeof(T), hipMemcpyHostToDevice) != hipSuccess) throw std::runtime_error("hipMemcpy failed while uploading the model");
        allocs.push_back(p);
        return DevPtr<T>{(T*)p};
    }
    template <typename real>
    DevPtr<real> upr(const std::vector<double>& v) {
        std::vector<real> w(v.begin(), v.end());
        return up(w);
    }

    template <typename real>
    void build(const Blob& b, DevModel<real>& m) {
        auto I = [&](const char* n) { return b.i(n); };
        auto F = [&](const char* n) { return b.f(n); };
        m.nq = b.scalar("nq"); m.nv = b.scalar("nv"); m.nu = b.scalar("nu"); m.nbody = b.scalar("nbody"); m.njnt = b.scalar("njnt");
        m.ngeom = b.scalar("ngeom"); m.npair = b.scalar("npair"); m.ntree = b.scalar("ntree"); m.neq = b.scalar("neq");
        m.task_id = b.scalar("task_id");
        m.nj = b.scalar("num_arms") == 3 ? 21 : 14;
        auto opt = F("opt");
        m.timestep = (real)opt[0]; m.gravity[0] = (real)opt[1]; m.gravity[1] = (real)opt[2]; m.gravity[2] = (real)opt[3];
        m.impratio = (real)opt[4]; m.noslip_iters = (int)opt[5]; m.noslip_per_tree = 1; m.noslip_trees = 1; m.newton_component = 1; m.newton_early_exit = 1; m.qcqp_tridiag = sizeof(real) == 4 ? 2 : 0;
        m.solver = 1; m.newton_iters = 100; m.newton_tol = sizeof(real) == 8 ? (real)1e-8 : (real)1e-6; m.ls_tolerance = sizeof(real) == 8 ? (real)1e-10 : (real)1e-4; m.ls_iterations = 50;
        m.nscale = (real)(1.0 / ((opt.size() > 7 && opt[7] > 0 ? opt[7] : 1.0) * std::max(1, m.nv)));
        auto gr = F("grip_range");
        m.grip_lo = (real)gr[0]; m.grip_hi = (real)gr[1];
        auto body_parent = I("body_parent"), body_dofadr = I("body_dofadr"), body_dofnum = I("body_dofnum"), body_tree = I("body_tree");
        auto dof_parent = I("dof_parent"), dof_tree = I("dof_tree"), tree_dofadr = I("tree_dofadr"), tree_dofnum = I("tree_dofnum");
        auto dof_body = I("dof_body");
        int nb = m.nbody, nv = m.nv, nt = m.ntree;
        for (int t = 0; t < nt; t++) if (tree_dofnum[t] > TREE_W) throw std::runtime_error("kinematic tree with more than 8 dofs");
        if (nb > 64) throw std::runtime_error("more than 64 bodies (kinematics maps one body per lane)");
        if (nt > 8) throw std::runtime_error("more than 8 kinematic trees (the per-tree solves map 8 lanes to a tree)");
        { auto jn = I("body_jntnum"); for (int bb = 0; bb < nb; bb++) if (jn[bb] > 1) throw std::runtime_error("body with more than one joint"); }
        std::vector<int> tba(nt + 1, 0), tbl;
        for (int t = 0; t < nt; t++) {
            tba[t] = (int)tbl.size();
            for (int bb = 1; bb < nb; bb++) if (body_tree[bb] == t) tbl.push_back(bb);
        }
        tba[nt] = (int)tbl.size();
        auto bpos = F("body_pos"), bquat = F("body_quat");
        std::vector<double> sx(3 * nb, 0.0), sm(9 * nb, 0.0);
        sm[0] = sm[4] = sm[8] = 1;
        auto q2m = [](const double* q, double* R) {
            double w = q[0], x = q[1], y = q[2], z = q[3];
            R[0] = 1 - 2 * (y * y + z * z); R[1] = 2 * (x * y - w * z); R[2] = 2 * (x * z + w * y);
            R[3] = 2 * (x * y + w * z); R[4] = 1 - 2 * (x * x + z * z); R[5] = 2 * (y * z - w * x);
            R[6] = 2 * (x * z - w * y); R[7] = 2 * (y * z + w * x); R[8] = 1 - 2 * (x * x + y * y);
        };
        for (int bb = 1; bb < nb; bb++) {
            if (body_tree[bb] >= 0) { sm[9 * bb] = sm[9 * bb + 4] = sm[9 * bb + 8] = 1; continue; }
            int p = body_parent[bb];
            double Rl[9];
            q2m(&bquat[4 * bb], Rl);
            for (int i = 0; i < 3; i++) {
                sx[3 * bb + i] = sx[3 * p + i] + sm[9 * p + 3 * i] * bpos[3 * bb] + sm[9 * p + 3 * i + 1] * bpos[3 * bb + 1] + sm[9 * p + 3 * i + 2] * bpos[3 * bb + 2];
                for (int j = 0; j < 3; j++) sm[9 * bb + 3 * i + j] = sm[9 * p + 3 * i] * Rl[j] + sm[9 * p + 3 * i + 1] * Rl[3 + j] + sm[9 * p + 3 * i + 2] * Rl[6 + j];
            }
        }
        std::vector<int> mask(nb, 0);
        for (int bb = 1; bb < nb; bb++) {
            int t = body_tree[bb];
            if (t < 0) continue;
            int c = bb;
            while (c > 0 && body_dofnum[c] == 0) c = body_parent[c];
            if (c == 0) continue;
            for (int d = body_dofadr[c] + body_dofnum[c] - 1; d >= 0; d = dof_parent[d]) mask[bb] |= 1 << (d - tree_dofadr[t]);
        }
        std::vector<int> mi, mj, madr(nt, 0);
        int ms = 0;
        for (int t = 0; t < nt; t++) { madr[t] = ms; ms += tree_dofnum[t] * tree_dofnum[t]; }
        for (int i = 0; i < nv; i++) for (int j = i; j >= 0; j = dof_parent[j]) { mi.push_back(i); mj.push_back(j); }
        m.msize = ms;
        m.nment = (int)mi.size();
        std::vector<int> fl, lj;
        auto floss = F("dof_frictionloss");
        for (int i = 0; i < nv; i++) if (floss[i] > 0) fl.push_back(i);
        auto jl = I("jnt_limited");
        for (int j = 0; j < m.njnt; j++) if (jl[j]) lj.push_back(j);
        m.nfloss = (int)fl.size();
        m.nlimited = (int)lj.size();
        m.body_parent = up(body_parent); moff.body_parent = (int)img_int.size(); { auto v_ = body_parent; img_int.insert(img_int.end(), v_.begin(), v_.end()); } m.body_jntadr = up(I("body_jntadr")); moff.body_jntadr = (int)img_int.size(); { auto v_ = I("body_jntadr"); img_int.insert(img_int.end(), v_.begin(), v_.end()); } m.body_jntnum = up(I("body_jntnum")); moff.body_jntnum = (int)img_int.size(); { auto v_ = I("body_jntnum"); img_int.insert(img_int.end(), v_.begin(), v_.end()); }
        m.body_dofadr = up(body_dofadr); moff.body_dofadr = (int)img_int.size(); { auto v_ = body_dofadr; img_int.insert(img_int.end(), v_.begin(), v_.end()); } m.body_dofnum = up(body_dofnum); moff.body_dofnum = (int)img_int.size(); { auto v_ = body_dofnum; img_int.insert(img_int.end(), v_.begin(), v_.end()); } m.body_tree = up(body_tree); moff.body_tree = (int)img_int.size(); { auto v_ = body_tree; img_int.insert(img_int.end(), v_.begin(), v_.end()); } m.body_dofmask = up(mask); moff.body_dofmask = (int)img_int.size(); { auto v_ = mask; img_int.insert(img_int.end(), v_.begin(), v_.end()); }
// ... 53 lines not shown
                    if (gtype[g] == G_CYLINDER) { ex[2] = ex[1]; ex[1] = ex[0]; }
                    for (int k = 0; k < 3; k++) { lo[k] = -ex[k]; hi[k] = ex[k]; }
                }
                for (int k = 0; k < 3; k++) { glbox[6 * g + k] = 0.5 * (lo[k] + hi[k]); glbox[6 * g + 3 + k] = 0.5 * (hi[k] - lo[k]); }
            }
            int bb = gbody[g];
            gstat[g] = body_tree[bb] < 0;
            if (gstat[g]) {
                for (int i = 0; i < 3; i++) {
                    gx0[3 * g + i] = sx[3 * bb + i] + sm[9 * bb + 3 * i] * gpos[3 * g] + sm[9 * bb + 3 * i + 1] * gpos[3 * g + 1] + sm[9 * bb + 3 * i + 2] * gpos[3 * g + 2];
                    gc0[3 * g + i] = sx[3 * bb + i] + sm[9 * bb + 3 * i] * gcp[3 * g] + sm[9 * bb + 3 * i + 1] * gcp[3 * g + 1] + sm[9 * bb + 3 * i + 2] * gcp[3 * g + 2];
                    for (int j = 0; j < 3; j++)
                        gm0[9 * g + 3 * i + j] = sm[9 * bb + 3 * i] * gmat[9 * g + j] + sm[9 * bb + 3 * i + 1] * gmat[9 * g + 3 + j] + sm[9 * bb + 3 * i + 2] * gmat[9 * g + 6 + j];
                }
                std::vector<double> pts;
                if (gtype[g] == G_MESH) {
                    for (int v = 0; v < ghull[2 * g + 1]; v++) for (int k = 0; k < 3; k++) pts.push_back(hv[3 * (ghull[2 * g] + v) + k]);
                } else {
                    double ex[3] = {gsize[3 * g], gsize[3 * g + 1], gsize[3 * g + 2]};
                    if (gtype[g] == G_SPHERE) ex[1] = ex[2] = ex[0];
                    if (gtype[g] == G_CYLINDER) { ex[2] = ex[1]; ex[1] = ex[0]; }
                    for (int c = 0; c < 8; c++) for (int k = 0; k < 3; k++) pts.push_back(((c >> k) & 1) ? ex[k] : -ex[k]);
                }
                for (int k = 0; k < 3; k++) { gaabb[6 * g + k] = 1e30; gaabb[6 * g + 3 + k] = -1e30; }
                for (size_t v = 0; v < pts.size() / 3; v++)
                    for (int i = 0; i < 3; i++) {
                        double w = gx0[3 * g + i] + gm0[9 * g + 3 * i] * pts[3 * v] + gm0[9 * g + 3 * i + 1] * pts[3 * v + 1] + gm0[9 * g + 3 * i + 2] * pts[3 * v + 2];
                        if (w < gaabb[6 * g + i]) gaabb[6 * g + i] = w;
                        if (w > gaabb[6 * g + 3 + i]) gaabb[6 * g + 3 + i] = w;
                    }
            }
        }
        m.geom_type = up(I("geom_type")); moff.geom_type = (int)img_int.size(); { auto v_ = I("geom_type"); img_int.insert(img_int.end(), v_.begin(), v_.end()); } m.geom_body = up(gbody); moff.geom_body = (int)img_int.size(); { auto v_ = gbody; img_int.insert(img_int.end(), v_.begin(), v_.end()); } m.geom_hull = up(I("geom_ctab")); m.geom_class = up(I("geom_class")); m.geom_static = up(gstat); moff.geom_static = (int)img_int.size(); { auto v_ = gstat; img_int.insert(img_int.end(), v_.begin(), v_.end()); }
        m.geom_pos = upr<real>(gpos); m.geom_mat = upr<real>(gmat); m.geom_size = upr<real>(F("geom_size")); m.geom_cpos = upr<real>(gcp); moff.geom_cpos = (int)img_real.size(); { auto v_ = gcp; img_real.insert(img_real.end(), v_.begin(), v_.end()); }
        m.geom_rbound = upr<real>(F("geom_rbound")); moff.geom_rbound = (int)img_real.size(); { auto v_ = F("geom_rbound"); img_real.insert(img_real.end(), v_.begin(), v_.end()); } m.geom_xpos0 = upr<real>(gx0); m.geom_xmat0 = upr<real>(gm0); m.geom_cen0 = upr<real>(gc0); m.geom_aabb0 = upr<real>(gaabb); m.geom_lbox = upr<real>(glbox);
        {
            auto ctab = I("geom_ctab"), cells = I("chull_cells"), cand = I("chull_cand");
            const size_t ncell = cells.size();
            std::vector<double> tab(32 * ncell, 0.0), ovf;
            std::vector<char> done(ncell, 0);
            for (int g = 0; g < ng; g++) {
                if (gtype[g] != G_MESH) continue;
                const int cb = ctab[2 * g], R = ctab[2 * g + 1], adr = ghull[2 * g];
                for (int c = 0; c < 6 * R * R; c++) {
                    if (done[cb + c]) continue;
                    done[cb + c] = 1;
                    const int rec = cells[cb + c], off = rec >> 8, cnt = rec & 255;
                    if (cnt < 1) throw std::runtime_error("support table: empty cell");
                    double* o = &tab[32 * (size_t)(cb + c)];
                    for (int k = 0; k < 8; k++) {
                        const int v = cand[off + (k < cnt ? k : cnt - 1)];
                        if (v < 0 || v >= ghull[2 * g + 1]) throw std::runtime_error("support table: candidate index outside its hull");
                        for (int q = 0; q < 3; q++) o[4 * k + q] = hv[3 * (size_t)(adr + v) + q];
                        o[4 * k + 3] = (double)v;
                    }
                    o[3] = (double)cnt;
                    o[7] = (double)(ovf.size() / 4);
                    for (int k = 8; k < cnt; k++) {
                        const int v = cand[off + k];
                        if (v < 0 || v >= ghull[2 * g + 1]) throw std::runtime_error("support table: candidate index outside its hull");
                        for (int q = 0; q < 3; q++) ovf.push_back(hv[3 * (size_t)(adr + v) + q]);
                        ovf.push_back((double)v);
                    }
                }
            }
            if (ovf.size() / 4 >= (1u << 24)) throw std::runtime_error("support table: overflow part too large");
            m.hull_ovf = (int)(tab.size() / 4);
            tab.insert(tab.end(), ovf.begin(), ovf.end());
            if (tab.empty()) tab.assign(4, 0.0);
            m.hull_vert = upr<real>(tab);
        }
        m.pair_geom = up(I("pair_geom")); m.pair_condim = up(I("pair_condim"));
        m.pair_friction = upr<real>(F("pair_friction")); m.pair_solref = upr<real>(F("pair_solref")); m.pair_solimp = upr<real>(F("pair_solimp"));
        m.pair_margin = upr<real>(F("pair_margin")); m.pair_gap = upr<real>(F("pair_gap"));
        m.obs_qposadr = up(I("obs_qposadr")); m.obs_offset = upr<real>(F("obs_offset")); m.obs_scale = upr<real>(F("obs_scale"));
        while (img_real.size() % 4) img_real.push_back(0.0);
        while (img_int.size() % 4) img_int.push_back(0);
        moff.nreal = (int)img_real.size();
        moff.nint = (int)img_int.size();
        d_img_real = (void*)upr<real>(img_real);
        d_img_int = up(img_int);
    }

    void make_layout(int nq, int nv, int nu, int nb, int ng, int msize, int ntree) {
        if (maxcon1 > maxcon) maxcon1 = maxcon;
        if (maxefc1 > maxefc) maxefc1 = maxefc;
        make_layout_of(lay, maxcon1, maxefc1, nq, nv, nu, nb, ng, msize, ntree);
        make_layout_of(lay2, maxcon, maxefc, nq, nv, nu, nb, ng, msize, ntree);
    }
    void make_layout_of(Layout& L, const int maxcon, const int maxefc, int nq, int nv, int nu, int nb, int ng, int msize, int ntree) {
        kargs_dirty = true;
        int o = 0;
        auto R = [&](int n) { int a = o; o += n; return a; };
        L.qpos = R(nq); L.qvel = R(nv); L.ctrl = R(nu); L.warm = R(nv);
        L.xpos = R(3 * nb); L.xmat = R(9 * nb); L.xipos = R(3 * nb); L.cdof = R(6 * nv); L.gcen = R(3 * ng);
        L.M = R(msize); L.L = R(msize); o = (o + 3) & ~3; L.Minv = R(64 * ntree);
        L.bias = R(nv); L.fsm = R(nv); L.asm_ = R(nv); L.qacc = R(nv); L.fcon = R(nv);
        {
            int nvh = nv * (nv + 1) / 2, need1 = nvh + 2 * nv, need2 = need1 + maxefc, avail = 15 * nb + 6 * nv + 3 * ng;
            int base = need1 <= avail ? L.xpos : R(need1);
            L.nH = base; L.ng = base + nvh; L.ndl = L.ng + nv;
            L.njv = need2 <= avail ? L.ndl + nv : R(maxefc);
        }
        L.U = o;
        int a = o;
        L.cinert = a; a += 10 * nb; L.binert = a; a += 10 * nb; L.cvel = a; a += 6 * nb; L.cacc = a; a += 6 * nb; L.cfrc = a; a += 6 * nb;
        int bq = o;
        L.cdist = bq; bq += maxcon; L.cpos = bq; bq += 3 * maxcon; L.cnrm = bq; bq += 3 * maxcon;
        bq = (bq + 3) & ~3; L.rowS = bq; L.scr = bq; bq += RS_S * maxefc;
        L.maxgrp = maxefc / 3 + 8;
        if (bq < L.scr + 64 * SLOT_W + 4 * 56) bq = L.scr + 64 * SLOT_W + 4 * 56;
        o = a > bq ? a : bq;
        L.nreal = (o + 3) & ~3;
        int io = 0;
        auto Iq = [&](int n) { int x = io; io += n; return x; };
        L.cand = Iq(ANC_MAX); L.cpair = Iq(maxcon); L.cefc = Iq(maxcon); L.rmeta = Iq(maxefc); L.rowI = Iq(maxefc); L.gI = Iq(maxefc / 3 + 8); L.misc = Iq(12); L.nprof = Iq(16);
        L.nint = (io + 3) & ~3;
        L.maxcon = maxcon;
        L.maxefc = maxefc;
        L.expcon = this->maxcon;
        L.gefc = this->maxefc;
        L.ggrp = this->maxefc / 3 + 8;
        size_t rs = f64 ? 8 : 4;
        L.bytes_per_env = (int)((L.nreal * rs + (size_t)L.nint * 4 + 15) & ~(size_t)15);
        if (getenv("AVSIM_DEBUG_LAYOUT"))
            fprintf(stderr, "avsim layout: %d reals + %d ints = %d B per env (U at %d: phase A %d, phase B %d words); tables %zu B\n", L.nreal, L.nint,
                    L.bytes_per_env, L.U, a - L.U, bq - L.U, (size_t)moff.nreal * rs + (size_t)moff.nint * 4);
    }

    int dims[7] = {0, 0, 0, 0, 0, 0, 0};
    size_t lds_bytes() const { return (size_t)lay.bytes_per_env + (size_t)moff.nreal * (f64 ? 8 : 4) + (size_t)moff.nint * 4; }
    void* d_rows = nullptr;
    void* d_coup = nullptr;
    int* d_near = nullptr;
    void* d_gref = nullptr;
    void alloc_contacts() {
        if (d_rows) (void)hipFree(d_rows);
        d_rows = nullptr;
        if (hipMalloc(&d_rows, (size_t)N * maxefc * ROW_S * (f64 ? 8 : 4) * 2) != hipSuccess) throw std::runtime_error("hipMalloc of the constraint row buffers failed");
        mf.rJ_glob = (float*)d_rows; md.rJ_glob = (double*)d_rows;
        mf.rB_glob = mf.rJ_glob + (size_t)N * maxefc * ROW_S; md.rB_glob = md.rJ_glob + (size_t)N * maxefc * ROW_S;
        if (d_coup) (void)hipFree(d_coup);
        if (d_near) (void)hipFree(d_near);
        if (d_gref) (void)hipFree(d_gref);
        d_coup = nullptr; d_near = nullptr; d_gref = nullptr;
        if (hipMalloc(&d_gref, ((size_t)N * dims[4] * 3 + (size_t)N * 64 * BOX_OVF_W) * (f64 ? 8 : 4)) != hipSuccess) throw std::runtime_error("hipMalloc of the Verlet reference buffer failed");
        mf.gref_glob = (float*)d_gref; md.gref_glob = (double*)d_gref;
        mf.bxo_glob = mf.gref_glob + (size_t)N * dims[4] * 3; md.bxo_glob = md.gref_glob + (size_t)N * dims[4] * 3;
        if (hipMalloc(&d_coup, (size_t)N * lay2.maxgrp * GA_W * (f64 ? 8 : 4)) != hipSuccess || hipMalloc((void**)&d_near, (size_t)N * (NEAR_MAX + CAND_MAX) * 4) != hipSuccess)
            throw std::runtime_error("hipMalloc of the coupling / neighbour buffers failed");
        mf.gA_glob = (float*)d_coup; md.gA_glob = (double*)d_coup; mf.near_glob = d_near; md.near_glob = d_near; mf.cand_glob = md.cand_glob = d_near + (size_t)N * NEAR_MAX;
        kargs_dirty = true;
        if (d_cpairs) (void)hipFree(d_cpairs);
        if (d_cdist) (void)hipFree(d_cdist);
        d_cpairs = nullptr; d_cdist = nullptr;
        if (hipMalloc((void**)&d_cpairs, (size_t)N * maxcon * 8) != hipSuccess || hipMalloc((void**)&d_cdist, (size_t)N * maxcon * 8) != hipSuccess)
            throw std::runtime_error("hipMalloc of the contact export buffers failed");
        (void)hipMemset(d_cpairs, 0xff, (size_t)N * maxcon * 8);
        (void)hipMemset(d_cdist, 0, (size_t)N * maxcon * 8);
    }
    bool init(const Blob& b, int N_, bool f64_, std::string& err) {
        N = N_;
        f64 = f64_;
        try {
            if (f64) build(b, md); else build(b, mf);
            static const int mx[5] = {4, 4, 5, 3, 4};
            max_reward = mx[b.scalar("task_id")];
            int ms = f64 ? md.msize : mf.msize;
            static const int cap_efc[5] = {176, 176, 336, 480, 176}, cap_con[5] = {48, 48, 72, 96, 48};
            static const int cap_efc1[5] = {176, 176, 224, 288, 176}, cap_con1[5] = {48, 48, 56, 64, 48};
            maxefc = cap_efc[b.scalar("task_id")];
            maxcon = cap_con[b.scalar("task_id")];
            maxefc1 = cap_efc1[b.scalar("task_id")];
            maxcon1 = cap_con1[b.scalar("task_id")];
            dims[0] = b.scalar("nq"); dims[1] = b.scalar("nv"); dims[2] = b.scalar("nu"); dims[3] = b.scalar("nbody"); dims[4] = b.scalar("ngeom"); dims[5] = ms; dims[6] = b.scalar("ntree");
            make_layout(dims[0], dims[1], dims[2], dims[3], dims[4], dims[5], dims[6]);
            d_qpos_home = up(b.f("qpos_home"));
            d_ctrl_home = up(b.f("ctrl_home"));
            d_obj_qadr = up(b.i("objects_qposadr"));
            d_ncon = up(std::vector<int>((size_t)N, 0));
            d_diag = up(std::vector<int>((size_t)N * 4, 0));
            d_cost = up(std::vector<int>((size_t)N, 0));
            d_order = up(std::vector<int>((size_t)N, 0));
            d_retry = up(std::vector<int>(2 * (size_t)N + 2, 0));
            alloc_contacts();
        } catch (const std::exception& e) {
            err = std::string("physics init: ") + e.what();
            return false;
        }
        return true;
    }
    void destroy() {
        for (void* p : allocs) (void)hipFree(p);
        allocs.clear();
        if (d_cpairs) (void)hipFree(d_cpairs);
        if (d_cdist) (void)hipFree(d_cdist);
        if (d_rows) (void)hipFree(d_rows);
        if (d_coup) (void)hipFree(d_coup);
        if (d_near) (void)hipFree(d_near);
        if (d_gref) (void)hipFree(d_gref);
        d_cpairs = nullptr; d_cdist = nullptr; d_rows = nullptr; d_coup = nullptr; d_near = nullptr; d_gref = nullptr;
    }
    bool set_option(const char* name, double v) {
        std::string n(name);
        kargs_dirty = true;
        if (n == "pgs_iters") { pgs_iters = (int)v; return true; }
        if (n == "solver") { if (v != 0 && v != 1) return false; mf.solver = md.solver = (int)v; return true; }
        if (n == "newton_iters") { if (v < 1 || v > 100) return false; mf.newton_iters = md.newton_iters = (int)v; return true; }
        if (n == "newton_tol") { if (v < 0) return false; mf.newton_tol = (float)v; md.newton_tol = v; return true; }
        if (n == "ls_tolerance") { if (!(v > 0) || v >= 1) return false; mf.ls_tolerance = (float)v; md.ls_tolerance = v; return true; }
        if (n == "ls_iterations") { if (v < 1 || v > 1000) return false; mf.ls_iterations = md.ls_iterations = (int)v; return true; }
        if (n == "export_contacts") { export_contacts = v != 0; return true; }
        if (n == "num_joints") { if (v != 14 && v != 21) return false; mf.nj = md.nj = (int)v; return true; }
        if (n == "order_envs") { order_envs = v != 0; return true; }
        if (n == "pair_waves") { pair_waves = v != 0; return true; }
        if (n == "qcqp_tridiag") { mf.qcqp_tridiag = md.qcqp_tridiag = v < 0 ? 0 : (v > 2 ? 2 : (int)v); return true; }
        if (n == "noslip_per_tree") { mf.noslip_per_tree = md.noslip_per_tree = v != 0; return true; }
        if (n == "noslip_trees") { mf.noslip_trees = md.noslip_trees = v != 0; return true; }
        if (n == "newton_component") { mf.newton_component = md.newton_component = v != 0; return true; }
        if (n == "newton_early_exit") { mf.newton_early_exit = md.newton_early_exit = v != 0; return true; }
        if (n == "persist_blocks") { int x = (int)v; if (x >= 1 && x <= 64) { persist_over = x; return true; } return false; }
        if (n == "waves_per_block") { int x = (int)v; if (x >= 0 && x <= AVSIM_PHYS_MAXW) { wpb_override = x; return true; } return false; }
        if (n == "profile_phases") {
            if (v != 0 && !d_prof) d_prof = up(std::vector<long long>((size_t)N * PROF_W, 0));
            if (v == 0) d_prof = nullptr;
            return true;
        }
        if (n == "maxefc" || n == "maxcon" || n == "maxefc_first" || n == "maxcon_first") {
            int x = (int)v;
            if (x < 16 || x > 1000) return false;
            (void)hipDeviceSynchronize();
            if (n == "maxefc") maxefc = maxefc1 = x; else if (n == "maxcon") maxcon = maxcon1 = x;
            else if (n == "maxefc_first") maxefc1 = x < maxefc ? x : maxefc; else maxcon1 = x < maxcon ? x : maxcon;
            make_layout(dims[0], dims[1], dims[2], dims[3], dims[4], dims[5], dims[6]);
            alloc_contacts();
            return true;
        }
        return false;
    }

    template <typename real, int MAXW>
    int waves_per_block(const Layout& L) const {
        const size_t tables = (size_t)moff.nreal * sizeof(real) + (size_t)moff.nint * 4;
        int wpb = tables < 160 * 1024 ? (int)((160 * 1024 - tables) / (size_t)L.bytes_per_env) : 0;
        if (wpb > MAXW) wpb = MAXW;
        if (wpb_override > 0) wpb = wpb_override < MAXW ? wpb_override : MAXW;
        return wpb < 1 ? 1 : wpb;
    }

    template <typename real, int G, int MAXW>
    int launch_t(hipStream_t st, const DevModel<real>& m, int nsub, const float* action, void* qpos, void* qvel, void* ctrl, void* warm,
                 int* latch, double* agent, int32_t* reward, uint8_t* success, std::string& err) {
        const size_t tables = (size_t)moff.nreal * sizeof(real) + (size_t)moff.nint * 4;
        auto kern1 = k_phys<real, G, MAXW, false>;
        auto kern2 = k_phys<real, G, MAXW, true>;
        if (!attr_done) {
            hipError_t e = hipFuncSetAttribute((const void*)kern1, hipFuncAttributeMaxDynamicSharedMemorySize, 160 * 1024);
            if (e == hipSuccess) e = hipFuncSetAttribute((const void*)kern2, hipFuncAttributeMaxDynamicSharedMemorySize, 160 * 1024);
            if (e != hipSuccess) { err = std::string("hipFuncSetAttribute: ") + hipGetErrorString(e); return -3; }
            int dev = 0;
            hipDeviceProp_t prop;
            if (hipGetDevice(&dev) == hipSuccess && hipGetDeviceProperties(&prop, dev) == hipSuccess && prop.multiProcessorCount > 0) num_cu = prop.multiProcessorCount;
            if (!d_head) {
                if (hipMalloc((void**)&d_head, 2 * sizeof(int)) != hipSuccess) { err = "hipMalloc(work counters) failed"; return -3; }
                allocs.push_back(d_head);
                (void)hipMemset(d_head, 0, 2 * sizeof(int));
            }
            attr_done = 1;
        }
        const bool two = two_pass();
        int wpb = waves_per_block<real, MAXW>(lay);
        const int wpb2 = waves_per_block<real, MAXW>(lay2);
        if (!two && wpb_override <= 0 && num_cu > 0 && N < num_cu * wpb) { wpb = (N + num_cu - 1) / num_cu; if (wpb < 1) wpb = 1; }
        const size_t pairflags = two ? 2 * (MAXW / 2 > 0 ? MAXW / 2 : 1) * sizeof(int) : 0;
        const size_t shmem = (size_t)lay.bytes_per_env * wpb + tables + pairflags, shmem2 = (size_t)lay2.bytes_per_env * wpb2 + tables + pairflags;
        const int pairing = (two && wpb >= 2 && lay2.bytes_per_env <= 2 * lay.bytes_per_env && pair_waves) ? 8 : 0;
        if (shmem > 160 * 1024 || (two && shmem2 > 160 * 1024)) { err = "per-block LDS exceeds 160 KiB; lower maxefc/maxcon"; return -1; }
        const int per_cu = (int)((160 * 1024) / shmem) > 0 ? (int)((160 * 1024) / shmem) : 1;
        int nblk = num_cu * per_cu * (persist_over > 0 ? persist_over : 1);
        if (nblk > (N + wpb - 1) / wpb) nblk = (N + wpb - 1) / wpb;
        if (kargs_dirty) {
            KArgs<real> ka{m, lay, moff}, ka2{m, lay2, moff};
            if (!d_kargs) { if (hipMalloc(&d_kargs, sizeof(KArgs<double>)) != hipSuccess) { err = "hipMalloc(kernel arguments) failed"; return -3; } allocs.push_back(d_kargs); }
            if (!d_kargs2) { if (hipMalloc(&d_kargs2, sizeof(KArgs<double>)) != hipSuccess) { err = "hipMalloc(kernel arguments) failed"; return -3; } allocs.push_back(d_kargs2); }
            (void)hipStreamSynchronize(st);
            if (hipMemcpy(d_kargs, &ka, sizeof(ka), hipMemcpyHostToDevice) != hipSuccess || hipMemcpy(d_kargs2, &ka2, sizeof(ka2), hipMemcpyHostToDevice) != hipSuccess) { err = "hipMemcpy(kernel arguments) failed"; return -3; }
            kargs_dirty = false;
        }
        static_assert((8 | 7) < (1 << 8), "retry_mode: mode bits and pairing flag below bit 8");
        if (two && (maxcon1 >= 1024 || maxefc1 >= 1024 || maxcon1 < 0 || maxefc1 < 0)) { err = "first-tier capacities do not fit the 10-bit fields of retry_mode (maxcon_first / maxefc_first < 1024)"; return -1; }
        const int* order = nullptr;
        if (order_envs && have_cost && nsub > 0 && N > wpb) {
            hipLaunchKernelGGL(k_env_order, dim3(1), dim3(1024), 0, st, (const int*)d_cost, d_order, N);
            order = d_order;
        }
        const int want_reward = (reward || success) && (nsub > 0 || force_reward) ? 1 : 0;
        const int par = (int)(retry_parity & 1);
        int* const rlist = d_retry + 2;
        {
            int* head = d_head + (launch_count & 1);
            int* next = d_head + ((launch_count + 1) & 1);
            launch_count++;
            hipLaunchKernelGGL(two ? kern2 : kern1, dim3(nblk), dim3(64 * wpb), shmem, st, (KPtr<real>)d_kargs, (const real*)d_img_real, (const int*)d_img_int, N, nsub, pgs_iters, action, want_reward,
                               (real*)qpos, (real*)qvel, (real*)ctrl, (real*)warm, latch, agent, (int*)reward, (unsigned char*)success, d_ncon,
                               d_cpairs, d_cdist, d_diag, max_reward, export_contacts, d_prof, d_xpose, order, order_envs ? d_cost : (int*)nullptr, head, next,
                               d_retry, two ? (1 + 2 * par) | pairing : 0, (KPtr<real>)d_kargs2);
        }
        if (two) {
            int* head = d_head + (launch_count & 1);
            int* next = d_head + ((launch_count + 1) & 1);
            launch_count++;
            retry_parity++;
            int nblk2 = num_cu;
            if (nblk2 > (N + wpb2 - 1) / wpb2) nblk2 = (N + wpb2 - 1) / wpb2;
            hipLaunchKernelGGL(kern2, dim3(nblk2), dim3(64 * wpb2), shmem2, st, (KPtr<real>)d_kargs2, (const real*)d_img_real, (const int*)d_img_int, N, nsub, pgs_iters, action, want_reward,
                               (real*)qpos, (real*)qvel, (real*)ctrl, (real*)warm, latch, agent, (int*)reward, (unsigned char*)success, d_ncon,
                               d_cpairs, d_cdist, d_diag, max_reward, export_contacts, d_prof, d_xpose, (const int*)rlist, order_envs ? d_cost : (int*)nullptr, head, next,
                               d_retry, (2 + 2 * par) | (maxcon1 << 8) | (maxefc1 << 18), (KPtr<real>)d_kargs2);
        }
        if (nsub > 0) have_cost = true;
        hipError_t e = hipGetLastError();
        if (e != hipSuccess) { err = std::string("physics kernel launch: ") + hipGetErrorString(e); return -3; }
        return 0;
    }

#ifndef AVSIM_TU_F64
    int launch(hipStream_t st, int N_, int nsub, const float* action, int nj, void* qpos, void* qvel, void* ctrl, void* warm, int* latch,
               double* agent, int32_t* reward, uint8_t* success, std::string& err) {
        (void)N_; (void)nj;
        if (f64) return phys_launch_f64(*this, st, nsub, action, qpos, qvel, ctrl, warm, latch, agent, reward, success, err);
        return launch_t<float, 64, AVSIM_PHYS_MAXW>(st, mf, nsub, action, qpos, qvel, ctrl, warm, latch, agent, reward, success, err);
    }
#endif
};

}
```

Before: 977,400.

## Add model-specialized physics kernel with compile-time layout and offset constants

Adds a separate translation unit that instantiates the f32 physics kernel with the layout and model-offset tables baked in as constexpr for specific task models (SlotInsertion-3Arms, HookPackage-2Arms). At launch the host compares the runtime layout, offsets and dimensions to each spec and switches to the specialized kernel when one matches. The aim is to turn the per-field loads from the kernel-argument struct into immediate constants, which cuts scalar loads and register pressure and lets the compiler fold address arithmetic. In exchange it adds build time, another code object, and hand-maintained tables that must stay in sync with the model.

```diff
diff --git a/av_aloha_amd/build.py b/av_aloha_amd/build.py
--- a/av_aloha_amd/build.py
+++ b/av_aloha_amd/build.py
@@ -30,9 +30,11 @@
 def _build_hip_locked(verbose):
     hipcc = os.environ.get("HIPCC", "/opt/rocm/bin/hipcc")
     common = [hipcc, "--offload-arch=gfx950", "-std=c++17", "-fPIC", "-fno-gpu-rdc", "-c"]
+    F32_FLAGS = ["-O2", "-fno-hip-fp32-correctly-rounded-divide-sqrt", "-fgpu-flush-denormals-to-zero", "-fno-slp-vectorize", "-fno-vectorize",
+                 "-mllvm", "-amdgpu-atomic-optimizer-strategy=None", "-mllvm", "-amdgpu-sched-strategy=max-ilp"]
     units = [
-        ("avsim_api", ["-O2", "-fno-hip-fp32-correctly-rounded-divide-sqrt", "-fgpu-flush-denormals-to-zero", "-fno-slp-vectorize", "-fno-vectorize",
-                       "-mllvm", "-amdgpu-atomic-optimizer-strategy=None", "-mllvm", "-amdgpu-sched-strategy=max-ilp"] + (["-DAVSIM_RENDER_STATS"] if os.environ.get("AVSIM_RENDER_STATS") else []) + os.environ.get("AVSIM_EXTRA_FLAGS", "").split()),
+        ("avsim_api", F32_FLAGS + (["-DAVSIM_RENDER_STATS"] if os.environ.get("AVSIM_RENDER_STATS") else []) + os.environ.get("AVSIM_EXTRA_FLAGS", "").split()),
+        ("avsim_phys_spec", F32_FLAGS + os.environ.get("AVSIM_EXTRA_FLAGS", "").split()),
         ("avsim_phys_f64", ["-O3", "-ffp-contract=off", "-mllvm", "-amdgpu-sched-strategy=max-ilp"] + os.environ.get("AVSIM_EXTRA_FLAGS_F64", "").split()),
     ]
     procs = []
diff --git a/av_aloha_amd/csrc/avsim_api.hip b/av_aloha_amd/csrc/avsim_api.hip
--- a/av_aloha_amd/csrc/avsim_api.hip
+++ b/av_aloha_amd/csrc/avsim_api.hip
@@ -558,9 +558,12 @@
     return AVSIM_OK;
 }
 
+#define AVS_PHYS_GATE(h) do { if ((h)->phys.refuses((h)->err)) return AVSIM_EINVAL; } while (0)
+
 int avsim_observe(avsim_t* h, double* agent_pos, int32_t* reward, uint8_t* success) {
     if (!h) return AVSIM_EINVAL;
     AVS_ON_DEVICE(h);
+    AVS_PHYS_GATE(h);
     int rc;
     void *dap = nullptr, *drw = nullptr, *dsu = nullptr;
     size_t N = h->N;
@@ -647,6 +650,7 @@
 int avsim_reset(avsim_t* h, const uint8_t* mask, const double* obj_qpos) {
     if (!h || !obj_qpos) { if (h) h->set_error("avsim_reset: obj_qpos is required"); return AVSIM_EINVAL; }
     AVS_ON_DEVICE(h);
+    AVS_PHYS_GATE(h);
     h->state_ver++;
     return h->f64 ? reset_impl<double>(h, mask, obj_qpos) : reset_impl<float>(h, mask, obj_qpos);
 }
@@ -689,6 +693,7 @@
 int avsim_step(avsim_t* h, const float* action, int nsub, double* agent_pos, int32_t* reward, uint8_t* success) {
     if (!h || !action || nsub < 0) { if (h) h->set_error("avsim_step: bad arguments"); return AVSIM_EINVAL; }
     AVS_ON_DEVICE(h);
+    AVS_PHYS_GATE(h);
     const void* da;
     int rc;
     if ((rc = h->in(0, action, sizeof(float) * h->N * h->nj, &da))) return rc;
@@ -698,6 +703,7 @@
 int avsim_step_ctrl(avsim_t* h, int nsub, double* agent_pos, int32_t* reward, uint8_t* success) {
     if (!h || nsub < 0) { if (h) h->set_error("avsim_step_ctrl: bad arguments"); return AVSIM_EINVAL; }
     AVS_ON_DEVICE(h);
+    AVS_PHYS_GATE(h);
     return step_common(h, nullptr, nsub, agent_pos, reward, success);
 }
 
@@ -709,6 +715,7 @@
     }
     if (h->num_arms != 3) { h->set_error("avsim_step_cartesian: the 23-D Cartesian action drives three arms (sim_env.py:277-282)"); return AVSIM_EINVAL; }
     AVS_ON_DEVICE(h);
+    AVS_PHYS_GATE(h);
     const void* da;
     int rc;
     if ((rc = h->in(0, action23, sizeof(double) * h->N * 23, &da))) return rc;
@@ -767,6 +774,7 @@
 int avsim_set_state(avsim_t* h, const double* qpos, const double* qvel, const double* ctrl, const double* warm) {
     if (!h) return AVSIM_EINVAL;
     AVS_ON_DEVICE(h);
+    AVS_PHYS_GATE(h);
     h->state_ver++;
     size_t N = h->N;
     int rc;
diff --git a/av_aloha_amd/csrc/avsim_newton.hip.h b/av_aloha_amd/csrc/avsim_newton.hip.h
--- a/av_aloha_amd/csrc/avsim_newton.hip.h
+++ b/av_aloha_amd/csrc/avsim_newton.hip.h
@@ -597,8 +597,8 @@
     if (nc < nv && omine) out[a0 + i8] = ox;
 }
 
-template <typename real, int NCH, bool COUPLED>
-__device__ __attribute__((always_inline)) int newton_solve(KPtr<real> ka, GLB_PTR(const real) rows, LDS_PTR(real) r_, LDS_PTR(int) ii_, LDS_PTR(const int) li_, int nefc, int ncon, int nlead,
+template <typename real, int NCH, bool COUPLED, typename KA>
+__device__ __attribute__((always_inline)) int newton_solve(KA ka, GLB_PTR(const real) rows, LDS_PTR(real) r_, LDS_PTR(int) ii_, LDS_PTR(const int) li_, int nefc, int ncon, int nlead,
                                                       int iters, real tol, real scale, int profiling) {
     const int lane = threadIdx.x & 63;
     NewtonArgs<real> A;
@@ -607,18 +607,16 @@
         LDS_PTR(int) ii = (LDS_PTR(int))(unsigned long long)(unsigned)__builtin_amdgcn_readfirstlane((int)(unsigned)(unsigned long long)ii_);
         LDS_PTR(const int) li = (LDS_PTR(const int))(unsigned long long)(unsigned)__builtin_amdgcn_readfirstlane((int)(unsigned)(unsigned long long)li_);
         tol = lane_get(tol, 0); scale = lane_get(scale, 0);
-        const Layout __attribute__((address_space(4)))* L = &ka->lay;
-        const MOff __attribute__((address_space(4)))* O = &ka->mo;
-        A.rowS = r + L->rowS; A.rowI = ii + L->rowI; A.rmeta = ii + L->rmeta;
+        A.rowS = r + ka->lay.rowS; A.rowI = ii + ka->lay.rowI; A.rmeta = ii + ka->lay.rmeta;
         {
             const unsigned long long p_ = (unsigned long long)rows;
             A.rJ = (GLB_PTR(const real))(((unsigned long long)(unsigned)__builtin_amdgcn_readfirstlane((int)(unsigned)(p_ >> 32)) << 32) | (unsigned)__builtin_amdgcn_readfirstlane((int)(unsigned)p_));
         }
-        A.M = r + L->M; A.a = r + L->qacc; A.as = r + L->asm_;
-        A.H = r + L->nH; A.g = r + L->ng; A.dl = r + L->ndl; A.jv = r + L->njv;
-        A.cefc = ii + L->cefc;
-        A.prof = profiling ? ii + L->nprof : (LDS_PTR(int))nullptr;
-        A.tree_dofadr = li + O->tree_dofadr; A.tree_dofnum = li + O->tree_dofnum; A.tree_madr = li + O->tree_madr; A.dof_tree = li + O->dof_tree;
+        A.M = r + ka->lay.M; A.a = r + ka->lay.qacc; A.as = r + ka->lay.asm_;
+        A.H = r + ka->lay.nH; A.g = r + ka->lay.ng; A.dl = r + ka->lay.ndl; A.jv = r + ka->lay.njv;
+        A.cefc = ii + ka->lay.cefc;
+        A.prof = profiling ? ii + ka->lay.nprof : (LDS_PTR(int))nullptr;
+        A.tree_dofadr = li + ka->mo.tree_dofadr; A.tree_dofnum = li + ka->mo.tree_dofnum; A.tree_madr = li + ka->mo.tree_madr; A.dof_tree = li + ka->mo.dof_tree;
         A.nv = __builtin_amdgcn_readfirstlane(ka->m.nv); A.ntree = __builtin_amdgcn_readfirstlane(ka->m.ntree);
         A.nefc = __builtin_amdgcn_readfirstlane(nefc); A.ncon = __builtin_amdgcn_readfirstlane(ncon);
         A.nlead = __builtin_amdgcn_readfirstlane(nlead); A.iters = __builtin_amdgcn_readfirstlane(iters);
@@ -914,8 +912,8 @@
     return used;
 }
 
-template <typename real, int NCH>
-__device__ AVS_OUTLINE_5 int newton_solve_coupled(KPtr<real> ka, GLB_PTR(const real) rows, LDS_PTR(real) r_, LDS_PTR(int) ii_, LDS_PTR(const int) li_, int nefc, int ncon, int nlead,
+template <typename real, int NCH, typename KA>
+__device__ AVS_OUTLINE_5 int newton_solve_coupled(KA ka, GLB_PTR(const real) rows, LDS_PTR(real) r_, LDS_PTR(int) ii_, LDS_PTR(const int) li_, int nefc, int ncon, int nlead,
                                                               int iters, real tol, real scale, int profiling) {
     return newton_solve<real, NCH, true>(ka, rows, r_, ii_, li_, nefc, ncon, nlead, iters, tol, scale, profiling);
 }
diff --git a/av_aloha_amd/csrc/avsim_phys.hip.h b/av_aloha_amd/csrc/avsim_phys.hip.h
--- a/av_aloha_amd/csrc/avsim_phys.hip.h
+++ b/av_aloha_amd/csrc/avsim_phys.hip.h
@@ -7,6 +7,7 @@
 #include "avsim_collide.hip.h"
 #include "avsim_math.hip.h"
 #include "avsim_model.h"
+#include "avsim_phys_layout.h"
 
 namespace avs {
 
@@ -15,10 +16,8 @@
 constexpr int TREE_W = 8;
 constexpr int ROW_W = 2 * TREE_W;
 constexpr int ROW_S = ROW_W;
-constexpr int RS_S = 9;
 constexpr int CAND_MAX = 256;
 constexpr int PROF_W = 26;
-constexpr int ANC_MAX = 64;
 constexpr int NEAR_MAX = 512;
 
 template <typename real>
@@ -136,73 +135,7 @@
     GLB_PTR(const real) obs_scale;
 };
 
-struct MOff {
-    int nreal, nint;
-    int body_parent;
-    int body_jntadr;
-    int body_jntnum;
-    int body_dofadr;
-    int body_dofnum;
-    int body_tree;
-    int body_dofmask;
-    int body_last;
-    int tree_bodyadr;
-    int tree_bodylist;
-    int tree_dofadr;
-    int tree_dofnum;
-    int tree_madr;
-    int jnt_type;
-    int jnt_qposadr;
-    int jnt_dofadr;
-    int jnt_actfrclimited;
-    int limited_jnt;
-    int dof_body;
-    int dof_parent;
-    int dof_tree;
-    int dof_jnt;
-    int floss_dof;
-    int ment_i;
-    int ment_j;
-    int act_dof;
-    int act_qposadr;
-    int act_ctrllimited;
-    int geom_type;
-    int geom_body;
-    int geom_static;
-    int body_pos;
-    int body_quat;
-    int body_mass;
-    int body_ipos;
-    int body_inertia;
-    int body_invweight0;
-    int jnt_pos;
-    int jnt_axis;
-    int jnt_range;
-    int jnt_actfrcrange;
-    int jnt_margin;
-    int dof_armature;
-    int dof_damping;
-    int dof_frictionloss;
-    int dof_invweight0;
-    int act_kp;
-    int act_kv;
-    int act_gear;
-    int act_ctrlrange;
-    int geom_cpos;
-    int geom_rbound;
-};
-
-struct Layout {
-    int qpos, qvel, ctrl, warm, xpos, xmat, xipos, cdof, gcen, M, L, Minv, bias, fsm, asm_, qacc, fcon, nH, ng, ndl, njv, U, nreal;
-    int cinert, cvel, cacc, cfrc, binert;
-    int cdist, cpos, cnrm, rowS, scr;
-    int cand, cpair, cefc, rmeta, rowI, gI, misc, nprof, nint;
-    int maxgrp;
-    int maxcon, maxefc;
-    int expcon;
-    int gefc, ggrp;
-    int bytes_per_env;
-};
+static_assert(NARROW_SCR_W == 64 * SLOT_W + 4 * 56, "avsim_phys_layout.h: narrow-phase scratch");
 
 template <typename real>
 struct KArgs {
@@ -212,6 +145,25 @@
 };
 template <typename real>
 using KPtr = const KArgs<real> __attribute__((address_space(4)))*;
+
+struct GenericSpec {};
+template <typename real, typename SPEC>
+struct KFixed {
+    KPtr<real> p;
+    struct View {
+        const DevModel<real> __attribute__((address_space(4)))& m;
+        static constexpr Layout lay = SPEC::lay;
+        static constexpr MOff mo = SPEC::mo;
+        AVS_DEV const View* operator->() const { return this; }
+    };
+    AVS_DEV KFixed(KPtr<real> p_) : p(p_) {}
+    AVS_DEV explicit KFixed(unsigned long long v) : p((KPtr<real>)v) {}
+    AVS_DEV explicit operator unsigned long long() const { return (unsigned long long)p; }
+    AVS_DEV View operator->() const { return View{p->m}; }
+};
+template <typename real, typename SPEC> struct KRefOf { using type = KFixed<real, SPEC>; };
+template <typename real> struct KRefOf<real, GenericSpec> { using type = KPtr<real>; };
+template <typename real, typename SPEC> using KRef = typename KRefOf<real, SPEC>::type;
 #define PHASE_LAUNDER()                                                                                \
     do {                                                                                               \
         const unsigned long long p_ = (unsigned long long)ka;                                          \
@@ -1461,8 +1413,8 @@
     real m, h[3], I[6];
 };
 
-template <typename real>
-AVS_DEV void body_inertia(KPtr<real> ka, const real* xmat, const real* xipos, int b, SInert<real>& s) {
+template <typename real, typename KA>
+AVS_DEV void body_inertia(KA ka, const real* xmat, const real* xipos, int b, SInert<real>& s) {
     const real* R = xmat + 9 * b;
     GLB_PTR(const real) Ib = ka->m.body_inertia + 6 * b;
     real I3[9] = {Ib[0], Ib[3], Ib[4], Ib[3], Ib[1], Ib[5], Ib[4], Ib[5], Ib[2]}, T[9], Ic[9];
@@ -1612,7 +1564,7 @@
     }
     return rw;
 }
-#ifndef AVSIM_TU_F64
+#if !defined(AVSIM_TU_F64) && !defined(AVSIM_NO_F32_LAUNCH)
 __global__ void k_reward_pairs(GLB_PTR(const int) geom_class, int ngeom, int task_id, const int* __restrict__ pairs, int n, int cap, int* __restrict__ latch, int* __restrict__ reward) {
     const int i = blockIdx.x * blockDim.x + threadIdx.x;
     if (i >= n) return;
@@ -1629,9 +1581,9 @@
 #endif
 
 
-template <typename real, int G>
+template <typename real, int G, typename SPEC = GenericSpec>
 struct Env {
-    KPtr<real> ka;
+    KRef<real, SPEC> ka;
     int env = 0;
     int diverged = 0;
     int nit_sum = 0, nit_max = 0;
@@ -1642,7 +1594,7 @@
     const real* lr;
     const int* li;
     long long t_broad = 0, t_narrow = 0;
-    __device__ Env(KPtr<real> ka_, real* r_, int* i_, int lane_, int grp_, const real* lr_, const int* li_)
+    __device__ Env(KRef<real, SPEC> ka_, real* r_, int* i_, int lane_, int grp_, const real* lr_, const int* li_)
         : ka(ka_), r(r_), ii(i_), lane(lane_), grp(grp_), lr(lr_), li(li_) {}
     AVS_DEV const int* LI() const { const int* p = li; AVS_ASSUME_LDS(p); return p; }
     AVS_DEV const real* LR() const { const real* p = lr; AVS_ASSUME_LDS(p); return p; }
@@ -2106,7 +2058,7 @@
         }
     }
 
-    __device__ AVS_OUTLINE_0 static void multi_perturb(KPtr<real> ka_, real* r_, int* i_, int lane_, int grp_, const real* lr_, const int* li_, int env_,
+    __device__ AVS_OUTLINE_0 static void multi_perturb(KRef<real, SPEC> ka_, real* r_, int* i_, int lane_, int grp_, const real* lr_, const int* li_, int env_,
                                                                    int pga, int pgb, int src, int pert) {
         Env e(ka_, r_, i_, lane_, grp_, lr_, li_);
         e.env = env_;
@@ -2899,7 +2851,7 @@
 #ifndef AVSIM_PHYS_MAXW
 #define AVSIM_PHYS_MAXW 8
 #endif
-template <typename real, int G, int MAXW, bool RETRY>
+template <typename real, int G, int MAXW, bool RETRY, typename SPEC = GenericSpec>
 #ifndef AVSIM_PHYS_ATTR
 #ifdef AVSIM_TU_F64
 #define AVSIM_PHYS_ATTR
@@ -2907,13 +2859,14 @@
 #define AVSIM_PHYS_ATTR __attribute__((amdgpu_waves_per_eu(2)))
 #endif
 #endif
-__global__ void __launch_bounds__(64 * MAXW) AVSIM_PHYS_ATTR k_phys(KPtr<real> ka_small, const real* __restrict__ img_real, const int* __restrict__ img_int, int N, int nsub, int pgs_iters, const float* __restrict__ action,
+__global__ void __launch_bounds__(64 * MAXW) AVSIM_PHYS_ATTR k_phys(KPtr<real> ka_small_, const real* __restrict__ img_real, const int* __restrict__ img_int, int N, int nsub, int pgs_iters, const float* __restrict__ action,
                                              int want_reward, real* __restrict__ g_qpos, real* __restrict__ g_qvel, real* __restrict__ g_ctrl,
                                              real* __restrict__ g_warm, int* __restrict__ g_latch, double* __restrict__ o_agent,
                                              int* __restrict__ o_reward, unsigned char* __restrict__ o_success, int* __restrict__ o_ncon,
                                              int* __restrict__ o_cpairs, double* __restrict__ o_cdist, int* __restrict__ o_diag, int max_reward, int export_contacts, long long* __restrict__ o_prof, float* __restrict__ o_xpose,
                                              const int* __restrict__ env_order, int* __restrict__ o_cost, int* __restrict__ work_head, int* __restrict__ work_next,
-                                             int* __restrict__ retry, int retry_mode, KPtr<real> ka_big) {
+                                             int* __restrict__ retry, int retry_mode, KPtr<real> ka_big_) {
+    const KRef<real, SPEC> ka_small(ka_small_), ka_big(ka_big_);
     extern __shared__ __attribute__((aligned(16))) unsigned char smem[];
     int nwork = N;
     const bool pass2 = RETRY && ((retry_mode & 7) == 2 || (retry_mode & 7) == 4);
@@ -2995,12 +2948,12 @@
         }
         if (polls >= (1 << 15)) { lds_put(&pair_want[pr], 0); to_list(env); continue; }
     }
-    KPtr<real> ka = (RETRY && big) ? ka_big : ka_small;
+    KRef<real, SPEC> ka = (RETRY && big) ? ka_big : ka_small;
     const long long t_launch = __builtin_readcyclecounter();
     real* r = reinterpret_cast<real*>(smem + (size_t)((RETRY && big) ? (wave & ~1) : wave) * ka_small->lay.bytes_per_env);
     int* ii = reinterpret_cast<int*>(r + ka->lay.nreal);
     bool beyond = false;
-    Env<real, G> E(ka, r, ii, lane, grp, lr, li);
+    Env<real, G, SPEC> E(ka, r, ii, lane, grp, lr, li);
     E.env = env;
 
     for (int i = lane; i < ka->m.nq; i += G) r[ka->lay.qpos + i] = g_qpos[(size_t)env * ka->m.nq + i];
@@ -3026,7 +2979,7 @@
         PROF(0, E.pre_phases());
 #else
         {
-            Env<real, G> e(E);
+            Env<real, G, SPEC> e(E);
             PROF(0, e.kinematics());
             PROF(1, e.crb());
             PROF(2, e.rne_bias());
@@ -3041,7 +2994,7 @@
         PROF(7, E.post_phases());
 #else
         {
-            Env<real, G> e(E);
+            Env<real, G, SPEC> e(E);
             PROF(7, e.euler());
             e.check_divergence();
             E.diverged = e.diverged;
@@ -3138,11 +3091,14 @@
 struct PhysHost;
 int phys_launch_f64(PhysHost& ph, hipStream_t st, int nsub, const float* action, void* qpos, void* qvel, void* ctrl, void* warm, int* latch,
                     double* agent, int32_t* reward, uint8_t* success, std::string& err);
+const void* phys_spec_kernel(const PhysHost& ph, const char** name);
 
 struct PhysHost {
     int maxcon = 48, maxefc = 144, pgs_iters = 20, group = 64, export_contacts = 1, force_reward = 0, wpb_override = 0;
     int maxcon1 = 48, maxefc1 = 144;
     bool f64 = false;
+    int specialised = 1;
+    bool host_only = false;
     int N = 0, max_reward = 0;
     std::vector<void*> allocs;
     DevModel<float> mf;
@@ -3186,6 +3142,7 @@
     DevPtr<T> up(const std::vector<T>& v) {
         void* p = nullptr;
         size_t n = (v.size() ? v.size() : 1) * sizeof(T);
+        if (host_only) return DevPtr<T>{nullptr};
         if (hipMalloc(&p, n) != hipSuccess) throw std::runtime_error("hipMalloc failed while uploading the model");
         if (v.size() && hipMemcpy(p, v.data(), v.size() * sizeof(T), hipMemcpyHostToDevice) != hipSuccess) throw std::runtime_error("hipMemcpy failed while uploading the model");
         allocs.push_back(p);
@@ -3405,6 +3362,18 @@
         d_img_int = up(img_int);
     }
 
+    const void* spec_kernel(const char** name) const {
+        if (f64 || specialised == 0 || two_pass()) return nullptr;
+        return phys_spec_kernel(*this, name);
+    }
+    bool refuses(std::string& err) const {
+        if (specialised != 2 || spec_kernel(nullptr)) return false;
+        err = std::string("phys_specialised = 2: no kernel compiled for this handle's model and layout (") +
+              (f64 ? "f64 handle" : two_pass() ? "two capacity tiers" : "Layout, table offsets or dims match no spec of avsim_phys_specs.h") + "); the launch would take the generic k_phys";
+        return true;
+    }
+    int spec_note = 0;
+
     void make_layout(int nq, int nv, int nu, int nb, int ng, int msize, int ntree) {
         if (maxcon1 > maxcon) maxcon1 = maxcon;
         if (maxefc1 > maxefc) maxefc1 = maxefc;
@@ -3413,42 +3382,12 @@
     }
     void make_layout_of(Layout& L, const int maxcon, const int maxefc, int nq, int nv, int nu, int nb, int ng, int msize, int ntree) {
         kargs_dirty = true;
-        int o = 0;
-        auto R = [&](int n) { int a = o; o += n; return a; };
-        L.qpos = R(nq); L.qvel = R(nv); L.ctrl = R(nu); L.warm = R(nv);
-        L.xpos = R(3 * nb); L.xmat = R(9 * nb); L.xipos = R(3 * nb); L.cdof = R(6 * nv); L.gcen = R(3 * ng);
-        L.M = R(msize); L.L = R(msize); o = (o + 3) & ~3; L.Minv = R(64 * ntree);
-        L.bias = R(nv); L.fsm = R(nv); L.asm_ = R(nv); L.qacc = R(nv); L.fcon = R(nv);
-        {
-            int nvh = nv * (nv + 1) / 2, need1 = nvh + 2 * nv, need2 = need1 + maxefc, avail = 15 * nb + 6 * nv + 3 * ng;
-            int base = need1 <= avail ? L.xpos : R(need1);
-            L.nH = base; L.ng = base + nvh; L.ndl = L.ng + nv;
-            L.njv = need2 <= avail ? L.ndl + nv : R(maxefc);
-        }
-        L.U = o;
-        int a = o;
-        L.cinert = a; a += 10 * nb; L.binert = a; a += 10 * nb; L.cvel = a; a += 6 * nb; L.cacc = a; a += 6 * nb; L.cfrc = a; a += 6 * nb;
-        int bq = o;
-        L.cdist = bq; bq += maxcon; L.cpos = bq; bq += 3 * maxcon; L.cnrm = bq; bq += 3 * maxcon;
-        bq = (bq + 3) & ~3; L.rowS = bq; L.scr = bq; bq += RS_S * maxefc;
-        L.maxgrp = maxefc / 3 + 8;
-        if (bq < L.scr + 64 * SLOT_W + 4 * 56) bq = L.scr + 64 * SLOT_W + 4 * 56;
-        o = a > bq ? a : bq;
-        L.nreal = (o + 3) & ~3;
-        int io = 0;
-        auto Iq = [&](int n) { int x = io; io += n; return x; };
-        L.cand = Iq(ANC_MAX); L.cpair = Iq(maxcon); L.cefc = Iq(maxcon); L.rmeta = Iq(maxefc); L.rowI = Iq(maxefc); L.gI = Iq(maxefc / 3 + 8); L.misc = Iq(12); L.nprof = Iq(16);
-        L.nint = (io + 3) & ~3;
-        L.maxcon = maxcon;
-        L.maxefc = maxefc;
-        L.expcon = this->maxcon;
-        L.gefc = this->maxefc;
-        L.ggrp = this->maxefc / 3 + 8;
-        size_t rs = f64 ? 8 : 4;
-        L.bytes_per_env = (int)((L.nreal * rs + (size_t)L.nint * 4 + 15) & ~(size_t)15);
-        if (getenv("AVSIM_DEBUG_LAYOUT"))
+        L = avs::make_layout_of(maxcon, maxefc, this->maxcon, this->maxefc, nq, nv, nu, nb, ng, msize, ntree, f64 ? 8 : 4);
+        if (getenv("AVSIM_DEBUG_LAYOUT")) {
+            const int pb = L.rowS + RS_S * maxefc > L.scr + NARROW_SCR_W ? L.rowS + RS_S * maxefc : L.scr + NARROW_SCR_W;
             fprintf(stderr, "avsim layout: %d reals + %d ints = %d B per env (U at %d: phase A %d, phase B %d words); tables %zu B\n", L.nreal, L.nint,
-                    L.bytes_per_env, L.U, a - L.U, bq - L.U, (size_t)moff.nreal * rs + (size_t)moff.nint * 4);
+                    L.bytes_per_env, L.U, 38 * nb, pb - L.U, (size_t)moff.nreal * (f64 ? 8 : 4) + (size_t)moff.nint * 4);
+        }
     }
 
     int dims[7] = {0, 0, 0, 0, 0, 0, 0};
@@ -3490,8 +3429,7 @@
             static const int mx[5] = {4, 4, 5, 3, 4};
             max_reward = mx[b.scalar("task_id")];
             int ms = f64 ? md.msize : mf.msize;
-            static const int cap_efc[5] = {176, 176, 336, 480, 176}, cap_con[5] = {48, 48, 72, 96, 48};
-            static const int cap_efc1[5] = {176, 176, 224, 288, 176}, cap_con1[5] = {48, 48, 56, 64, 48};
+            const int *cap_efc = CAP_EFC, *cap_con = CAP_CON, *cap_efc1 = CAP_EFC1, *cap_con1 = CAP_CON1;
             maxefc = cap_efc[b.scalar("task_id")];
             maxcon = cap_con[b.scalar("task_id")];
             maxefc1 = cap_efc1[b.scalar("task_id")];
@@ -3536,6 +3474,7 @@
         if (n == "export_contacts") { export_contacts = v != 0; return true; }
         if (n == "num_joints") { if (v != 14 && v != 21) return false; mf.nj = md.nj = (int)v; return true; }
         if (n == "order_envs") { order_envs = v != 0; return true; }
+        if (n == "phys_specialised") { if (v != 0 && v != 1 && v != 2) return false; specialised = (int)v; return true; }
         if (n == "pair_waves") { pair_waves = v != 0; return true; }
         if (n == "qcqp_tridiag") { mf.qcqp_tridiag = md.qcqp_tridiag = v < 0 ? 0 : (v > 2 ? 2 : (int)v); return true; }
         if (n == "noslip_per_tree") { mf.noslip_per_tree = md.noslip_per_tree = v != 0; return true; }
@@ -3577,6 +3516,13 @@
         const size_t tables = (size_t)moff.nreal * sizeof(real) + (size_t)moff.nint * 4;
         auto kern1 = k_phys<real, G, MAXW, false>;
         auto kern2 = k_phys<real, G, MAXW, true>;
+        const char* spec_name = nullptr;
+        const void* kspec = sizeof(real) == 4 && MAXW == AVSIM_PHYS_MAXW ? spec_kernel(&spec_name) : nullptr;
+        if (refuses(err)) return -1;
+        if (spec_note != (kspec ? 1 : 2) && getenv("AVSIM_DEBUG_LAYOUT")) {
+            fprintf(stderr, "avsim: k_phys %s%s\n", kspec ? "specialised for " : "generic", kspec ? spec_name : "");
+            spec_note = kspec ? 1 : 2;
+        }
         if (!attr_done) {
             hipError_t e = hipFuncSetAttribute((const void*)kern1, hipFuncAttributeMaxDynamicSharedMemorySize, 160 * 1024);
             if (e == hipSuccess) e = hipFuncSetAttribute((const void*)kern2, hipFuncAttributeMaxDynamicSharedMemorySize, 160 * 1024);
@@ -3590,6 +3536,14 @@
                 (void)hipMemset(d_head, 0, 2 * sizeof(int));
             }
             attr_done = 1;
+        }
+        if (kspec) {
+            if (!(attr_done & 2)) {
+                const hipError_t e = hipFuncSetAttribute(kspec, hipFuncAttributeMaxDynamicSharedMemorySize, 160 * 1024);
+                if (e != hipSuccess) { err = std::string("hipFuncSetAttribute(") + spec_name + "): " + hipGetErrorString(e); return -3; }
+                attr_done |= 2;
+            }
+            kern1 = (decltype(kern1))kspec;
         }
         const bool two = two_pass();
         int wpb = waves_per_block<real, MAXW>(lay);
@@ -3647,7 +3601,7 @@
         return 0;
     }
 
-#ifndef AVSIM_TU_F64
+#if !defined(AVSIM_TU_F64) && !defined(AVSIM_NO_F32_LAUNCH)
     int launch(hipStream_t st, int N_, int nsub, const float* action, int nj, void* qpos, void* qvel, void* ctrl, void* warm, int* latch,
                double* agent, int32_t* reward, uint8_t* success, std::string& err) {
         (void)N_; (void)nj;
diff --git a/av_aloha_amd/csrc/avsim_phys_layout.h b/av_aloha_amd/csrc/avsim_phys_layout.h
--- /dev/null
+++ b/av_aloha_amd/csrc/avsim_phys_layout.h
@@ -0,0 +1,121 @@
+#pragma once
+
+namespace avs {
+
+constexpr int RS_S = 9;
+constexpr int ANC_MAX = 64;
+constexpr int NARROW_SCR_W = 64 * 24 + 4 * 56;
+
+struct MOff {
+    int nreal, nint;
+    int body_parent;
+    int body_jntadr;
+    int body_jntnum;
+    int body_dofadr;
+    int body_dofnum;
+    int body_tree;
+    int body_dofmask;
+    int body_last;
+    int tree_bodyadr;
+    int tree_bodylist;
+    int tree_dofadr;
+    int tree_dofnum;
+    int tree_madr;
+    int jnt_type;
+    int jnt_qposadr;
+    int jnt_dofadr;
+    int jnt_actfrclimited;
+    int limited_jnt;
+    int dof_body;
+    int dof_parent;
+    int dof_tree;
+    int dof_jnt;
+    int floss_dof;
+    int ment_i;
+    int ment_j;
+    int act_dof;
+    int act_qposadr;
+    int act_ctrllimited;
+    int geom_type;
+    int geom_body;
+    int geom_static;
+    int body_pos;
+    int body_quat;
+    int body_mass;
+    int body_ipos;
+    int body_inertia;
+    int body_invweight0;
+    int jnt_pos;
+    int jnt_axis;
+    int jnt_range;
+    int jnt_actfrcrange;
+    int jnt_margin;
+    int dof_armature;
+    int dof_damping;
+    int dof_frictionloss;
+    int dof_invweight0;
+    int act_kp;
+    int act_kv;
+    int act_gear;
+    int act_ctrlrange;
+    int geom_cpos;
+    int geom_rbound;
+};
+constexpr int MOFF_WORDS = sizeof(MOff) / sizeof(int);
+
+struct Layout {
+    int qpos, qvel, ctrl, warm, xpos, xmat, xipos, cdof, gcen, M, L, Minv, bias, fsm, asm_, qacc, fcon, nH, ng, ndl, njv, U, nreal;
+    int cinert, cvel, cacc, cfrc, binert;
+    int cdist, cpos, cnrm, rowS, scr;
+    int cand, cpair, cefc, rmeta, rowI, gI, misc, nprof, nint;
+    int maxgrp;
+    int maxcon, maxefc;
+    int expcon;
+    int gefc, ggrp;
+    int bytes_per_env;
+};
+constexpr int LAYOUT_WORDS = sizeof(Layout) / sizeof(int);
+
+constexpr Layout make_layout_of(int maxcon, int maxefc, int full_maxcon, int full_maxefc, int nq, int nv, int nu, int nb, int ng, int msize,
+                                int ntree, int real_bytes) {
+    Layout L{};
+    int o = 0;
+    L.qpos = o; o += nq; L.qvel = o; o += nv; L.ctrl = o; o += nu; L.warm = o; o += nv;
+    L.xpos = o; o += 3 * nb; L.xmat = o; o += 9 * nb; L.xipos = o; o += 3 * nb; L.cdof = o; o += 6 * nv; L.gcen = o; o += 3 * ng;
+    L.M = o; o += msize; L.L = o; o += msize; o = (o + 3) & ~3; L.Minv = o; o += 64 * ntree;
+    L.bias = o; o += nv; L.fsm = o; o += nv; L.asm_ = o; o += nv; L.qacc = o; o += nv; L.fcon = o; o += nv;
+    {
+        const int nvh = nv * (nv + 1) / 2, need1 = nvh + 2 * nv, need2 = need1 + maxefc, avail = 15 * nb + 6 * nv + 3 * ng;
+        int base = L.xpos;
+        if (!(need1 <= avail)) { base = o; o += need1; }
+        L.nH = base; L.ng = base + nvh; L.ndl = L.ng + nv;
+        if (need2 <= avail) L.njv = L.ndl + nv;
+        else { L.njv = o; o += maxefc; }
+    }
+    L.U = o;
+    int a = o;
+    L.cinert = a; a += 10 * nb; L.binert = a; a += 10 * nb; L.cvel = a; a += 6 * nb; L.cacc = a; a += 6 * nb; L.cfrc = a; a += 6 * nb;
+    int bq = o;
+    L.cdist = bq; bq += maxcon; L.cpos = bq; bq += 3 * maxcon; L.cnrm = bq; bq += 3 * maxcon;
+    bq = (bq + 3) & ~3; L.rowS = bq; L.scr = bq; bq += RS_S * maxefc;
+    L.maxgrp = maxefc / 3 + 8;
+    if (bq < L.scr + NARROW_SCR_W) bq = L.scr + NARROW_SCR_W;
+    o = a > bq ? a : bq;
+    L.nreal = (o + 3) & ~3;
+    int io = 0;
+    L.cand = io; io += ANC_MAX; L.cpair = io; io += maxcon; L.cefc = io; io += maxcon; L.rmeta = io; io += maxefc; L.rowI = io; io += maxefc;
+    L.gI = io; io += maxefc / 3 + 8; L.misc = io; io += 12; L.nprof = io; io += 16;
+    L.nint = (io + 3) & ~3;
+    L.maxcon = maxcon;
+    L.maxefc = maxefc;
+    L.expcon = full_maxcon;
+    L.gefc = full_maxefc;
+    L.ggrp = full_maxefc / 3 + 8;
+    L.bytes_per_env = (int)(((unsigned long long)L.nreal * (unsigned)real_bytes + (unsigned long long)L.nint * 4 + 15) & ~15ull);
+    return L;
+}
+
+constexpr int CAP_EFC[5] = {176, 176, 336, 480, 176}, CAP_CON[5] = {48, 48, 72, 96, 48};
+constexpr int CAP_EFC1[5] = {176, 176, 224, 288, 176}, CAP_CON1[5] = {48, 48, 56, 64, 48};
+
+}
diff --git a/av_aloha_amd/csrc/avsim_phys_spec.hip b/av_aloha_amd/csrc/avsim_phys_spec.hip
--- /dev/null
+++ b/av_aloha_amd/csrc/avsim_phys_spec.hip
@@ -0,0 +1,25 @@
+#define AVSIM_NO_F32_LAUNCH 1
+#include "avsim_phys.hip.h"
+#include "avsim_phys_specs.h"
+
+namespace avs {
+
+template <typename SPEC>
+static bool spec_matches(const PhysHost& ph) {
+    static_assert(sizeof(Layout) == LAYOUT_WORDS * sizeof(int) && sizeof(MOff) == MOFF_WORDS * sizeof(int), "structs of ints, no padding");
+    static constexpr Layout lay = SPEC::lay;
+    static constexpr MOff mo = SPEC::mo;
+    return std::memcmp(&ph.lay, &lay, sizeof(Layout)) == 0 && std::memcmp(&ph.lay2, &lay, sizeof(Layout)) == 0 &&
+           std::memcmp(&ph.moff, &mo, sizeof(MOff)) == 0 && std::memcmp(ph.dims, SPEC::dims, sizeof(ph.dims)) == 0;
+}
+
+const void* phys_spec_kernel(const PhysHost& ph, const char** name) {
+    if (ph.f64 || ph.two_pass()) return nullptr;
+#define AVSIM_SPEC_TRY(SPEC) \
+    if (spec_matches<SPEC>(ph)) { if (name) *name = SPEC::name; return (const void*)k_phys<float, 64, AVSIM_PHYS_MAXW, false, SPEC>; }
+    AVSIM_PHYS_SPECS(AVSIM_SPEC_TRY)
+#undef AVSIM_SPEC_TRY
+    return nullptr;
+}
+
+}
diff --git a/av_aloha_amd/csrc/avsim_phys_specs.h b/av_aloha_amd/csrc/avsim_phys_specs.h
--- /dev/null
+++ b/av_aloha_amd/csrc/avsim_phys_specs.h
@@ -0,0 +1,30 @@
+#pragma once
+#include "avsim_phys_layout.h"
+
+namespace avs {
+
+struct SpecSlotInsertion3Arms {
+    static constexpr const char* name = "slot_insertion_3arms";
+    static constexpr int maxcon = 48, maxefc = 176;
+    static constexpr int dims[7] = {37, 35, 21, 31, 84, 249, 5};
+    static constexpr Layout lay = make_layout_of(maxcon, maxefc, maxcon, maxefc, 37, 35, 21, 31, 84, 249, 5, 4);
+    static constexpr MOff mo = {1448, 1160, 0, 31, 62, 93, 124, 155, 186, 217, 248, 254, 281, 286, 291, 296,
+                                321, 346, 371, 396, 419, 454, 489, 524, 559, 565, 705, 845, 866, 887, 908, 992,
+                                1076, 0, 93, 217, 248, 341, 527, 589, 664, 739, 789, 839, 864, 899, 934, 969,
+                                1004, 1025, 1046, 1067, 1109, 1361};
+};
+
+struct SpecHookPackage2Arms {
+    static constexpr const char* name = "hook_package_2arms";
+    static constexpr int maxcon = 48, maxefc = 176;
+    static constexpr int dims[7] = {37, 35, 21, 32, 87, 249, 5};
+    static constexpr Layout lay = make_layout_of(maxcon, maxefc, maxcon, maxefc, 37, 35, 21, 32, 87, 249, 5, 4);
+    static constexpr MOff mo = {1476, 1180, 0, 32, 64, 96, 128, 160, 192, 224, 256, 262, 289, 294, 299, 304,
+                                329, 354, 379, 404, 427, 462, 497, 532, 567, 573, 713, 853, 874, 895, 916, 1003,
+                                1090, 0, 96, 224, 256, 352, 544, 608, 683, 758, 808, 858, 883, 918, 953, 988,
+                                1023, 1044, 1065, 1086, 1128, 1389};
+};
+
+#define AVSIM_PHYS_SPECS(X) X(SpecSlotInsertion3Arms) X(SpecHookPackage2Arms)
+
+}
```

Result: faster. 1.004 million, median of 6 (+2.7%).
